# ActiveVisionLab/DFNet

Hardware: AMD Instinct MI355X
Metric: rendered rays/sec (64+128 samples, 640x480) (higher is better)
Workload: dtype f16x3; 1 GPU; BASELINE configs[1]: synthetic random-weight NeRF-H (D=8, W=128), 640x480, 64+128 samples, test-time render_image, 1 frame per step per GPU; parallelism=frames sharded over 1 GPU(s), gather at end, collectives=none (one rank)

## Files before the change

### dfnet_amd/csrc/nerfh_api.hip

```cpp
#include <hip/hip_runtime.h>

#include <cmath>
#include <cstdarg>
#include <cstdio>
#include <cstdlib>
#include <cstring>
#include <map>
#include <string>
#include <type_traits>
#include <vector>

#include "../../include/dfnet_hip.h"
#include "dfn_common.h"
#include "nerfh_fused_train.h"
#include "nerfh_handle.h"
#include "nerfh_kernels.h"
#include "nerfh_layout.h"

using namespace dfn;

namespace dfn {
static thread_local char g_err[512] = "";
int set_error(int code, const char* fmt, ...) {
  va_list ap;
  va_start(ap, fmt);
  vsnprintf(g_err, sizeof g_err, fmt, ap);
  va_end(ap);
  return code;
}
int device_cu_count() {
  static int n = 0;
  if (!n) {
    int dev = 0;
    hipDeviceProp_t p;
    if (hipGetDevice(&dev) == hipSuccess && hipGetDeviceProperties(&p, dev) == hipSuccess) n = p.multiProcessorCount;
    if (n <= 0) n = 256;
  }
  return n;
}
}

extern "C" const char* dfn_last_error(void) { return g_err; }
extern "C" int dfn_abi_version(void) { return 1; }

static std::map<std::string, std::vector<size_t>> expected_shapes(const dfn_nerfh_desc& d) {
  std::map<std::string, std::vector<size_t>> m;
  const size_t W = d.width, na = size_t(d.hist_bin) * d.dim_a, nt = size_t(d.hist_bin) * d.dim_t;
  for (int f = 0; f < 2; ++f) {
    const std::string pre = f ? "fine." : "coarse.";
    for (int i = 0; i < d.depth; ++i) {
      const size_t k = i == 0 ? kChXyz : (i == 4 ? W + kChXyz : W);
      m[pre + "xyz_encoding_" + std::to_string(i + 1) + ".0.weight"] = {W, k};
      m[pre + "xyz_encoding_" + std::to_string(i + 1) + ".0.bias"] = {W};
    }
    m[pre + "xyz_encoding_final.weight"] = {W, W};
    m[pre + "xyz_encoding_final.bias"] = {W};
    m[pre + "dir_encoding.0.weight"] = {W / 2, W + kChDir + (f ? na : 0)};
    m[pre + "dir_encoding.0.bias"] = {W / 2};
    m[pre + "static_sigma.0.weight"] = {1, W};
    m[pre + "static_sigma.0.bias"] = {1};
    m[pre + "static_rgb.0.weight"] = {3, W / 2};
    m[pre + "static_rgb.0.bias"] = {3};
    if (f) {
      const size_t ks[4] = {W + nt, W / 2, W / 2, W / 2};
      for (int j = 0; j < 4; ++j) {
        m[pre + "transient_encoding." + std::to_string(2 * j) + ".weight"] = {W / 2, ks[j]};
        m[pre + "transient_encoding." + std::to_string(2 * j) + ".bias"] = {W / 2};
      }
      m[pre + "transient_sigma.0.weight"] = {1, W / 2};
      m[pre + "transient_sigma.0.bias"] = {1};
      m[pre + "transient_rgb.0.weight"] = {3, W / 2};
      m[pre + "transient_rgb.0.bias"] = {3};
      m[pre + "transient_beta.0.weight"] = {1, W / 2};
      m[pre + "transient_beta.0.bias"] = {1};
    }
  }
  m["embedding_a.weight"] = {size_t(d.n_vocab), size_t(d.dim_a)};
  m["embedding_t.weight"] = {size_t(d.n_vocab), size_t(d.dim_t)};
  return m;
}

extern "C" int dfn_nerfh_create(const dfn_nerfh_desc* desc, dfn_nerfh_t* out) {
  if (!desc || !out) return set_error(DFN_ERR_ARG, "dfn_nerfh_create: null argument");
  if (desc->depth != 8 || desc->multires != kLxyz || desc->multires_views != kLdir)
    return set_error(DFN_ERR_UNSUPPORTED,
                     "dfn_nerfh_create: kernels are specialised for netdepth=8 multires=%d multires_views=%d (got %d/%d/%d)",
                     kLxyz, kLdir, desc->depth, desc->multires, desc->multires_views);
  if (desc->width < 2 || desc->width > 1024 || (desc->width & 1))
    return set_error(DFN_ERR_UNSUPPORTED, "dfn_nerfh_create: netwidth must be even and in [2, 1024] (got %d)", desc->width);
  if (desc->hist_bin <= 0 || desc->dim_a <= 0 || desc->dim_t <= 0 || desc->n_vocab <= 0 ||
      desc->hist_bin * (desc->dim_a + desc->dim_t) > 1024)
    return set_error(DFN_ERR_ARG, "dfn_nerfh_create: bad embedding geometry");
  auto* h = new dfn_nerfh_s();
  h->desc = *desc;
  *out = h;
  return DFN_OK;
}

static void free_packed(dfn_nerfh_s* h) {
  for (auto& a : h->net)
    for (auto& b : a)
      for (auto& n : b) {
        if (n.blob) (void)hipFree(n.blob);
        if (n.tab) (void)hipFree(n.tab);
        n = PackedNet();
      }
  for (auto& n : h->bwd) {
    if (n.blob) (void)hipFree(n.blob);
    if (n.tab) (void)hipFree(n.tab);
    n = PackedNet();
  }
  if (h->extra) (void)hipFree(h->extra);
  h->extra = nullptr;
  if (h->gen_blob) (void)hipFree(h->gen_blob);
  h->gen_blob = nullptr;
  h->gen_params.clear();
  h->fast = false;
}

extern "C" int dfn_nerfh_destroy(dfn_nerfh_t h) {
  if (!h) return DFN_OK;
  free_packed(h);
  dfn::fused::destroy_state(h);
  for (hipEvent_t e : h->side_ev) if (e) (void)hipEventDestroy(e);
  if (h->side_stream) (void)hipStreamDestroy(h->side_stream);
  if (h->range_flag) (void)hipFree(h->range_flag);
  delete h;
  return DFN_OK;
}

extern "C" int dfn_nerfh_set_param(dfn_nerfh_t h, const char* name, const float* host, size_t numel) {
  if (!h || !name || !host) return set_error(DFN_ERR_ARG, "dfn_nerfh_set_param: null argument");
  const auto shapes = expected_shapes(h->desc);
  const auto it = shapes.find(name);
  if (it == shapes.end()) return set_error(DFN_ERR_ARG, "dfn_nerfh_set_param: unknown parameter '%s'", name);
  size_t want = 1;
  for (size_t s : it->second) want *= s;
  if (want != numel)
    return set_error(DFN_ERR_ARG, "dfn_nerfh_set_param: '%s' has %zu elements, expected %zu", name, numel, want);
  h->params[name].assign(host, host + numel);
  h->committed = false;
  return DFN_OK;
}

namespace {

struct Mat {
  const float* w = nullptr;
  const float* b = nullptr;
  int rows = 0, cols = 0;
};

struct Packer {
  const dfn_nerfh_s* h;
  std::string pre;
  int width() const { return h->desc.width; }
  mutable int fwd_units = 0;
  std::vector<float> fold_dir, fold_tr;
  Mat mat(const std::string& key) const {
    Mat m;
    const auto& w = h->params.at(pre + key + ".weight");
    const auto& b = h->params.at(pre + key + ".bias");
    m.w = w.data();
    m.b = b.data();
    m.rows = int(b.size());
    m.cols = int(w.size() / b.size());
    return m;
  }
  void row_source(int layer, int mb, int i, Mat& m, int& row) const {
    row = 32 * mb + i;
    switch (layer) {
      case LY_L1: case LY_L2: case LY_L3: case LY_L4: case LY_L5: case LY_L6: case LY_L7: case LY_L8:
        m = mat("xyz_encoding_" + std::to_string(layer - LY_L1 + 1) + ".0");
        break;
      case LY_FIN:
        if (mb < width() / 32) m = mat("xyz_encoding_final");
        else { m = mat("static_sigma.0"); row = i == 0 ? 0 : -1; }
        break;
      case LY_DIR: m = mat("dir_encoding.0"); break;
      case LY_RGB: m = mat("static_rgb.0"); row = i < 3 ? i : -1; break;
      case LY_TE0: m = mat("transient_encoding.0"); break;
      case LY_TE1: m = mat("transient_encoding.2"); break;
      case LY_TE2: m = mat("transient_encoding.4"); break;
      case LY_TE3: m = mat("transient_encoding.6"); break;
      case LY_THEAD:
        if (i < 3) { m = mat("transient_rgb.0"); row = i; }
        else if (i == 3) { m = mat("transient_sigma.0"); row = 0; }
        else if (i == 8) { m = mat("transient_beta.0"); row = 0; }
        else { m = mat("transient_beta.0"); row = -1; }
        break;
      case LY_SIG: m = mat("static_sigma.0"); row = i == 0 ? 0 : -1; break;
      case LY_DIRF: case LY_TE0F:
        m = Mat();
        m.w = (layer == LY_DIRF ? fold_dir : fold_tr).data();
        m.rows = width() / 2;
        m.cols = width();
        break;
    }
  }
  static int col_source(int layer, int hh, int s) {
    if (layer == LY_L1) return pe_xyz_feature(hh, s);
    if (layer == LY_L5) return s < 32 ? pe_xyz_feature(hh, s) : kChXyz + hidden_feature(hh, s - 32);
    return hidden_feature(hh, s);
  }
  static int col_source_m16(int layer, int g, int s) {
    if (layer == LY_L1) return pe_xyz_feature_m16(g, s);
    if (layer == LY_L5) return s < 16 ? pe_xyz_feature_m16(g, s) : kChXyz + hidden_feature_m16(g, s - 16);
    return hidden_feature_m16(g, s);
  }
  bool head_block(int layer, int mb) const {
    return layer == LY_RGB || layer == LY_THEAD || layer == LY_SIG || (layer == LY_FIN && mb == width() / 32);
  }
  int row_m16(int layer, int mb, int i) const { return head_block(layer, mb) ? head_row_m16(i) : i; }
  static bool unit_has_bias(int layer) { return layer != LY_DIR && layer != LY_TE0 && layer != LY_DIRF && layer != LY_TE0F; }

  float wscale = 1.f;
  template <class P>
  void pack_blocks(int layer, int mb0, int group, uint8_t* base) const {
    using Elem = typename std::conditional<P::kSlotsPerChunk == 8, _Float16, float>::type;
    const LayerShape sh = layer_shape(layer, width());
    const int KC = sh.slots / P::kSlotsPerChunk;
    Elem* frag = reinterpret_cast<Elem*>(base);
    float* bias = reinterpret_cast<float*>(base + size_t(group) * KC * 64 * P::kLaneBytes);
    for (int g = 0; g < group; ++g) {
      const int mb = mb0 + g;
      if constexpr (P::kM16) {
        auto source = [&](int i, Mat& m, int& row) {
          const int ri = row_m16(layer, mb, i);
          if (ri < 0) { m = Mat(); row = -1; return; }
          row_source(layer, mb, ri, m, row);
          if (row >= m.rows) row = -1;
        };
        for (int lane = 0; lane < 64; ++lane)
          for (int kc = 0; kc < KC; ++kc) {
            Mat m;
            int row;
            source(16 * (kc & 1) + (lane & 15), m, row);
            for (int j = 0; j < 8; ++j) {
              const int col = col_source_m16(layer, lane >> 4, 8 * (kc >> 1) + j);
              const float v = (row >= 0 && col >= 0 && col < m.cols) ? m.w[size_t(row) * m.cols + col] : 0.f;
              Elem* fr = frag + (size_t(g) * KC + kc) * 64 * 16;
              const Elem hi = Elem(v * wscale);
              fr[lane * 8 + j] = hi;
              fr[512 + lane * 8 + j] = Elem(v * wscale - float(hi));
            }
          }
        for (int lg = 0; lg < 4; ++lg)
          for (int ms = 0; ms < 2; ++ms)
            for (int r = 0; r < 4; ++r) {
              Mat m;
              int row;
              source(16 * ms + 4 * lg + r, m, row);
              const float b = (row >= 0 && unit_has_bias(layer)) ? m.b[row] : 0.f;
              bias[g * 32 + lg * 8 + ms * 4 + r] = b * wscale * kX3ActScale;
            }
        continue;
      }
      for (int lane = 0; lane < 64; ++lane) {
        const int i = lane & 31, hh = lane >> 5;
        Mat m;
        int row;
        row_source(layer, mb, i, m, row);
        if (row >= m.rows) row = -1;
        for (int kc = 0; kc < KC; ++kc)
          for (int j = 0; j < P::kSlotsPerChunk; ++j) {
            const int col = col_source(layer, hh, kc * P::kSlotsPerChunk + j);
            const float v = (row >= 0 && col >= 0 && col < m.cols) ? m.w[size_t(row) * m.cols + col] : 0.f;
            if constexpr (P::kSplit) {
              Elem* fr = frag + (size_t(g) * KC + kc) * 64 * 16;
              const Elem hi = Elem(v * wscale);
              fr[lane * 8 + j] = hi;
              fr[512 + lane * 8 + j] = Elem(v * wscale - float(hi));
            } else {
              frag[((size_t(g) * KC + kc) * 64 + lane) * P::kSlotsPerChunk + j] = Elem(v);
            }
          }
      }
      for (int hh = 0; hh < 2; ++hh)
        for (int r = 0; r < 16; ++r) {
          Mat m;
          int row;
          row_source(layer, mb, mblock_row(hh, r), m, row);
          if (row >= m.rows) row = -1;
          const float b = (row >= 0 && unit_has_bias(layer)) ? m.b[row] : 0.f;
          bias[(g * 2 + hh) * 16 + r] = P::kSplit ? b * wscale * kX3ActScale : b;
        }
    }
  }
  float bwd_elem(int layer, int mb, int i, int hh, int s) const {
    const int k = 32 * mb + i;
    auto W = [](const Mat& m, int row, int col) {
      return (row >= 0 && row < m.rows && col >= 0 && col < m.cols) ? m.w[size_t(row) * m.cols + col] : 0.f;
    };
    auto pe_col = [&](int blk) { return pe_xyz_feature(mblock_half_of_row(i), 16 * blk + mblock_reg_of_row(i)); };
    const int j = hidden_feature(hh, s);
    switch (layer) {
      case BW_THEAD:
        if (j < 3) return W(mat("transient_rgb.0"), j, k);
        if (j == 3) return W(mat("transient_sigma.0"), 0, k);
        if (j == 8) return W(mat("transient_beta.0"), 0, k);
        return 0.f;
      case BW_TE3: return W(mat("transient_encoding.6"), j, k);
      case BW_TE2: return W(mat("transient_encoding.4"), j, k);
      case BW_TE1: return W(mat("transient_encoding.2"), j, k);
      case BW_RGB: return j < 3 ? W(mat("static_rgb.0"), j, k) : 0.f;
      case BW_FINCAT: {
        const bool dirpart = s >= 32;
        const int jj = hidden_feature(hh, s & 31);
        if (mb < 4) return W(mat(dirpart ? "dir_encoding.0" : "transient_encoding.0"), jj, k);
        if (!dirpart) return 0.f;
        const int c = pe_dir_feature(mblock_half_of_row(i), mblock_reg_of_row(i));
        return c >= 0 ? W(mat("dir_encoding.0"), jj, kWidth + c) : 0.f;
      }
      case BW_FIN:
        if (s < 64) return W(mat("xyz_encoding_final"), j, k);
        return (s == 64 && hh == 0) ? W(mat("static_sigma.0"), 0, k) : 0.f;
      case BW_L5:
        if (mb < 4) return W(mat("xyz_encoding_5.0"), j, kChXyz + k);
        return W(mat("xyz_encoding_5.0"), j, pe_col(mb - 4));
      case BW_L1: return W(mat("xyz_encoding_1.0"), j, pe_col(mb));
      default: {
        const int n = 8 - (layer - BW_L8);
        return W(mat("xyz_encoding_" + std::to_string(n) + ".0"), j, k);
      }
    }
  }
  template <class P>
  void pack_bwd_blocks(int layer, int mb0, int group, uint8_t* base) const {
    using Elem = typename std::conditional<P::kSlotsPerChunk == 8, _Float16, float>::type;
    const LayerShape sh = bwd_layer_shape(layer);
    const int KC = sh.slots / P::kSlotsPerChunk;
    Elem* frag = reinterpret_cast<Elem*>(base);
    for (int g = 0; g < group; ++g)
      for (int lane = 0; lane < 64; ++lane)
        for (int kc = 0; kc < KC; ++kc)
          for (int j = 0; j < P::kSlotsPerChunk; ++j) {
            const float v = bwd_elem(layer, mb0 + g, lane & 31, lane >> 5, kc * P::kSlotsPerChunk + j);
            if constexpr (P::kSplit) {
              Elem* fr = frag + (size_t(g) * KC + kc) * 64 * 16;
              const Elem hi = Elem(v * wscale);
              fr[lane * 8 + j] = hi;
              fr[512 + lane * 8 + j] = Elem(v * wscale - float(hi));
            } else {
              frag[((size_t(g) * KC + kc) * 64 + lane) * P::kSlotsPerChunk + j] = Elem(v);
            }
          }
  }
  template <class PF, class P>
  void pack_bwd(std::vector<uint8_t>& blob, std::vector<uint32_t>& tab) const {
    pack<PF>(true, bwd_fwd_unit_mb<PF>(), false, blob, tab);
    fwd_units = int(tab.size() / 2);
    const int umb = bwd_unit_mb<P>();
    for (int layer = 0; layer < BW_COUNT; ++layer) {
      const LayerShape sh = bwd_layer_shape(layer);
      for (int u0 = 0; u0 < sh.mb; u0 += umb) {
        const int mb0 = (umb <= 2 && layer == BW_L5) ? (u0 < 2 ? 4 + u0 : u0 - 2) : u0;
        const int group = sh.mb - mb0 < umb ? sh.mb - mb0 : umb;
        const uint32_t bytes = unit_bytes<P>(sh.slots, group);
        const uint32_t off = uint32_t(blob.size());
        blob.resize(off + bytes, 0);
        tab.push_back(off);
        tab.push_back(bytes);
        pack_bwd_blocks<P>(layer, mb0, group, blob.data() + off);
      }
    }
  }

  template <class P>
  uint32_t blocks_bytes(int layer, int group) const {
    const LayerShape sh = layer_shape(layer, width());
    return uint32_t(group) * (sh.slots / P::kSlotsPerChunk) * 64 * P::kLaneBytes + uint32_t(group) * 128;
  }

  template <class P>
  void pack(bool fine, int umb, bool merge, std::vector<uint8_t>& blob, std::vector<uint32_t>& tab, int l5_umb = -1, bool fold = false) const {
    const int* seq = fine ? (fold ? kFineFoldSeq : kFineSeq) : kCoarseSeq;
    const int* grp = fine ? kFineGroup : kCoarseGroup;
    const int nl = fine ? kFineLayers : kCoarseLayers;
    if (merge) {
      for (int li = 0; li < nl;) {
        int lj = li;
        uint32_t bytes = 0;
        while (lj < nl && grp[lj] == grp[li]) bytes += blocks_bytes<P>(seq[lj], layer_shape(seq[lj], width()).mb), ++lj;
        if (seq[li] == LY_L5) {
          const LayerShape sh = layer_shape(LY_L5, width());
          const int g = l5_unit_mb(umb);
          for (int mb0 = 0; mb0 < sh.mb; mb0 += g) {
            const uint32_t ub = unit_bytes<P>(sh.slots, g), uo = uint32_t(blob.size());
            blob.resize(uo + ub, 0);
            tab.push_back(uo);
            tab.push_back(ub);
            pack_blocks<P>(LY_L5, mb0, g, blob.data() + uo);
          }
          li = lj;
          continue;
        }
        const uint32_t off = uint32_t(blob.size());
        blob.resize(off + align_piece(bytes), 0);
        tab.push_back(off);
        tab.push_back(align_piece(bytes));
        uint32_t at = off;
        for (int l = li; l < lj; ++l) {
          pack_blocks<P>(seq[l], 0, layer_shape(seq[l], width()).mb, blob.data() + at);
          at += blocks_bytes<P>(seq[l], layer_shape(seq[l], width()).mb);
        }
        li = lj;
      }
      return;
    }
    for (int li = 0; li < nl; ++li) {
      const LayerShape sh = layer_shape(seq[li], width());
      const int lu = (seq[li] == LY_L5 && l5_umb > 0) ? l5_umb : umb;
      for (int mb0 = 0; mb0 < sh.mb; mb0 += lu) {
        const int group = sh.mb - mb0 < lu ? sh.mb - mb0 : lu;
        const uint32_t bytes = unit_bytes<P>(sh.slots, group);
        const uint32_t off = uint32_t(blob.size());
        blob.resize(off + bytes, 0);
        tab.push_back(off);
        tab.push_back(bytes);
        pack_blocks<P>(seq[li], mb0, group, blob.data() + off);
      }
    }
  }
};

void fold_final(const std::vector<float>& a, int rows, int lda, const std::vector<float>& F, const std::vector<float>& bF, int W,
                std::vector<float>& af, std::vector<float>& ab) {
  af.assign(size_t(rows) * W, 0.f);
  ab.assign(rows, 0.f);
  std::vector<double> acc(W);
  for (int r = 0; r < rows; ++r) {
    std::fill(acc.begin(), acc.end(), 0.0);
    double b = 0.0;
    for (int k = 0; k < W; ++k) {
      const double ark = a[size_t(r) * lda + k];
      const float* frow = &F[size_t(k) * W];
      for (int c = 0; c < W; ++c) acc[c] += ark * double(frow[c]);
      b += ark * double(bF[k]);
    }
    for (int c = 0; c < W; ++c) af[size_t(r) * W + c] = float(acc[c]);
    ab[r] = float(b);
  }
}

int upload(const void* src, size_t bytes, void** dst) {
  if (hipMalloc(dst, bytes ? bytes : 16) != hipSuccess) return set_error(DFN_ERR_HIP, "hipMalloc(%zu) failed", bytes);
  if (bytes && hipMemcpy(*dst, src, bytes, hipMemcpyHostToDevice) != hipSuccess)
    return set_error(DFN_ERR_HIP, "hipMemcpy H2D (%zu bytes) failed", bytes);
  return DFN_OK;
}

}

__global__ void range_fetch_kernel(int* flag) { flag[1] = atomicExch(flag, 0); }

extern "C" int dfn_nerfh_set_render_options(dfn_nerfh_t h, int flags) {
  if (!h) return set_error(DFN_ERR_ARG, "dfn_nerfh_set_render_options: null handle");
  if (flags & ~(DFN_RENDER_LINDISP | DFN_RENDER_COARSE_F16)) return set_error(DFN_ERR_UNSUPPORTED, "dfn_nerfh_set_render_options: unknown option bits 0x%x", flags);
  h->render_flags = flags;
  return DFN_OK;
}

extern "C" int dfn_nerfh_range_status(dfn_nerfh_t h, int* flags, void* stream) {
  if (!h) return set_error(DFN_ERR_ARG, "dfn_nerfh_range_status: null handle");
  int v = 0;
  if (h->range_flag) {
    hipStream_t s = static_cast<hipStream_t>(stream);
    hipLaunchKernelGGL(range_fetch_kernel, dim3(1), dim3(1), 0, s, h->range_flag);
    if (hipGetLastError() != hipSuccess || hipMemcpyAsync(&v, h->range_flag + 1, sizeof(int), hipMemcpyDeviceToHost, s) != hipSuccess ||
        hipStreamSynchronize(s) != hipSuccess)
      return set_error(DFN_ERR_HIP, "dfn_nerfh_range_status: reading the flag failed");
  }
  if (flags) { *flags = v; return DFN_OK; }
  if (v)
    return set_error(DFN_ERR_RANGE, "NeRF-H render: activations left the range of the %s arithmetic since the last check (%s); the frames rendered "
                     "since then are not the network's output: render them with DFN_PREC_F32",
                     (v & DFN_RANGE_F16_OVERFLOW) ? "f16" : "split-f16",
                     (v & DFN_RANGE_F16_OVERFLOW) ? "an f16 layer output overflowed to inf: |activation| > 65504"
                                                  : "a split-f16 hi half saturated: |activation| >= 4094 (hidden layers of the render kernels: "
                                                    ">= 4094 x the network's largest |weight|, the accumulators are narrowed before they are scaled)");
  return DFN_OK;
}

extern "C" int dfn_nerfh_range_status_async(dfn_nerfh_t h, int* host_flags, void* stream) {
  if (!h || !host_flags) return set_error(DFN_ERR_ARG, "dfn_nerfh_range_status_async: null handle / destination");
  if (!h->range_flag) { *host_flags = 0; return DFN_OK; }
  hipStream_t s = static_cast<hipStream_t>(stream);
  hipLaunchKernelGGL(range_fetch_kernel, dim3(1), dim3(1), 0, s, h->range_flag);
  if (hipGetLastError() != hipSuccess || hipMemcpyAsync(host_flags, h->range_flag + 1, sizeof(int), hipMemcpyDeviceToHost, s) != hipSuccess)
    return set_error(DFN_ERR_HIP, "dfn_nerfh_range_status_async: enqueueing the read failed");
  return DFN_OK;
}

extern "C" int dfn_nerfh_commit(dfn_nerfh_t h) {
  if (!h) return set_error(DFN_ERR_ARG, "dfn_nerfh_commit: null handle");
  for (const auto& kv : expected_shapes(h->desc))
    if (!h->params.count(kv.first)) return set_error(DFN_ERR_STATE, "dfn_nerfh_commit: parameter '%s' not set", kv.first.c_str());
  free_packed(h);
  dfn::fused::destroy_state(h);
  if (!h->range_flag) {
    if (hipMalloc(reinterpret_cast<void**>(&h->range_flag), 3 * sizeof(int)) != hipSuccess) {
      h->range_flag = nullptr;
      return set_error(DFN_ERR_HIP, "dfn_nerfh_commit: allocating the range-guard flag failed");
    }
    if (hipMemset(h->range_flag, 0, 3 * sizeof(int)) != hipSuccess) return set_error(DFN_ERR_HIP, "dfn_nerfh_commit: clearing the range-guard flag failed");
  }
  {
    std::vector<float> all;
    std::vector<size_t> offs;
    const int np = dfn_nerfh_train_param_count();
    for (int i = 0; i < np; ++i) {
      const auto& v = h->params.at(dfn_nerfh_train_param_name(i));
      offs.push_back(all.size());
      all.insert(all.end(), v.begin(), v.end());
      all.resize((all.size() + 3) & ~size_t(3));
    }
    int rc = upload(all.data(), all.size() * 4, reinterpret_cast<void**>(&h->gen_blob));
    if (rc) return rc;
    for (size_t o : offs) h->gen_params.push_back(h->gen_blob + o);
  }
  const int Wd = h->desc.width;
  std::vector<float> fold_bd, fold_bt;
  if (Wd != kWidth && Wd != kMaxWidth) {
    h->committed = true;
    return DFN_OK;
  }
  if (Wd == kMaxWidth) {
    for (int f = 0; f < 2; ++f)
      for (int prec = 0; prec < 3; ++prec) {
        Packer pk{h, f ? "fine." : "coarse."};
        std::vector<uint8_t> blob;
        std::vector<uint32_t> tab;
        PackedNet& n = h->net[f][prec][0];
        if (prec == DFN_PREC_F16) pk.pack<PrecF16>(f, unit_mb_w256<PrecF16>(), false, blob, tab);
        else if (prec == DFN_PREC_F32) pk.pack<PrecF32>(f, unit_mb_w256<PrecF32>(), false, blob, tab);
        else {
          float wmax = 0.f;
          for (const auto& kv : h->params)
            if (kv.first.compare(0, pk.pre.size(), pk.pre) == 0 && kv.first.find(".weight") != std::string::npos)
              for (float v : kv.second) wmax = std::fmax(wmax, std::fabs(v));
          int sexp = wmax > 0.f ? -int(std::ceil(std::log2(wmax))) : 0;
          sexp = sexp < -8 ? -8 : (sexp > 24 ? 24 : sexp);
          pk.wscale = std::ldexp(1.f, sexp);
          n.in_scale = pk.wscale * kX3ActScale;
          pk.pack<PrecX3>(f, unit_mb_w256<PrecX3>(), false, blob, tab);
        }
        int rc = upload(blob.data(), blob.size(), reinterpret_cast<void**>(&n.blob));
        if (rc) return rc;
        rc = upload(tab.data(), tab.size() * 4, reinterpret_cast<void**>(&n.tab));
        if (rc) return rc;
        n.n_units = int(tab.size() / 2);
      }
  } else {
  for (int f = 0; f < 2; ++f)
    for (int prec = 0; prec < 3; ++prec)
      for (int var = 0; var < kVariants; ++var) {
        const bool fold = var == kFoldVariant;
        if (fold && !(f == 1 && prec == DFN_PREC_F16X3)) continue;
        Packer pk{h, f ? "fine." : "coarse."};
        std::vector<uint8_t> blob;
        std::vector<uint32_t> tab;
        PackedNet& n = h->net[f][prec][var];
        if (prec == DFN_PREC_F16) pk.pack<PrecF16>(f, unit_mb<PrecF16>(var), unit_mb<PrecF16>(var) >= 8, blob, tab);
        else if (prec == DFN_PREC_F32) pk.pack<PrecF32>(f, unit_mb<PrecF32>(var), false, blob, tab);
        else {
          float wmax = 0.f;
          for (const auto& kv : h->params)
            if (kv.first.compare(0, pk.pre.size(), pk.pre) == 0 && kv.first.find(".weight") != std::string::npos)
              for (float v : kv.second) wmax = std::fmax(wmax, std::fabs(v));
          int sexp = wmax > 0.f ? -int(std::ceil(std::log2(wmax))) : 0;
          sexp = sexp < -8 ? -8 : (sexp > 24 ? 24 : sexp);
          pk.wscale = std::ldexp(1.f, sexp);
          n.in_scale = pk.wscale * kX3ActScale;
          if (fold) {
            const int ldd = Wd + kChDir + h->desc.hist_bin * h->desc.dim_a, ldt = Wd + h->desc.hist_bin * h->desc.dim_t;
            const auto& F = h->params.at("fine.xyz_encoding_final.weight");
            const auto& bF = h->params.at("fine.xyz_encoding_final.bias");
            fold_final(h->params.at("fine.dir_encoding.0.weight"), Wd / 2, ldd, F, bF, Wd, pk.fold_dir, fold_bd);
            fold_final(h->params.at("fine.transient_encoding.0.weight"), Wd / 2, ldt, F, bF, Wd, pk.fold_tr, fold_bt);
            pk.pack<PrecX3M16>(f, unit_mb<PrecX3M16>(var), false, blob, tab, l5_unit_mb_p<PrecX3M16>(unit_mb<PrecX3M16>(var)), true);
          } else if (var == 4) pk.pack<PrecX3M16>(f, unit_mb<PrecX3M16>(var), false, blob, tab, l5_unit_mb_p<PrecX3M16>(unit_mb<PrecX3M16>(var)));
          else pk.pack<PrecX3>(f, unit_mb<PrecX3>(var), false, blob, tab, l5_unit_mb_p<PrecX3>(unit_mb<PrecX3>(var)));
        }
        int rc = upload(blob.data(), blob.size(), reinterpret_cast<void**>(&n.blob));
        if (rc) return rc;
        rc = upload(tab.data(), tab.size() * 4, reinterpret_cast<void**>(&n.tab));
        if (rc) return rc;
        n.n_units = int(tab.size() / 2);
      }
  for (int prec = 0; prec < 3; ++prec) {
    Packer pk{h, "fine."};
    std::vector<uint8_t> blob;
    std::vector<uint32_t> tab;
    PackedNet& n = h->bwd[prec];
    if (prec == DFN_PREC_F16) pk.pack_bwd<PrecF16, PrecF16>(blob, tab);
    else if (prec == DFN_PREC_F32) pk.pack_bwd<PrecF32, PrecF32>(blob, tab);
    else {
      n.in_scale = h->net[1][2][0].in_scale * 1024.f;
      pk.wscale = n.in_scale / kX3ActScale;
      pk.pack_bwd<PrecX3, PrecX3>(blob, tab);
    }
    int rc = upload(blob.data(), blob.size(), reinterpret_cast<void**>(&n.blob));
    if (rc) return rc;
    rc = upload(tab.data(), tab.size() * 4, reinterpret_cast<void**>(&n.tab));
    if (rc) return rc;
    n.n_units = int(tab.size() / 2);
    n.n_fwd_units = pk.fwd_units;
  }
  }
  const dfn_nerfh_desc& d = h->desc;
  const int na = d.hist_bin * d.dim_a, nt = d.hist_bin * d.dim_t, kd = kChDir + na, NO = Wd / 2;
  const auto& wd = h->params.at("fine.dir_encoding.0.weight");
  const auto& bd = h->params.at("fine.dir_encoding.0.bias");
  const auto& wt = h->params.at("fine.transient_encoding.0.weight");
  const auto& bt = h->params.at("fine.transient_encoding.0.bias");
  const auto& ea = h->params.at("embedding_a.weight");
  const auto& et = h->params.at("embedding_t.weight");
  std::vector<float> ex;
  const size_t o_wd = 0, o_bd = o_wd + size_t(kd) * NO, o_wt = o_bd + NO, o_bt = o_wt + size_t(nt) * NO,
               o_ea = o_bt + NO, o_et = o_ea + ea.size(), o_bdf = o_et + et.size(), o_btf = o_bdf + NO;
  ex.resize(o_btf + NO);
  const int ld_d = Wd + kd, ld_t = Wd + nt;
  for (int j = 0; j < kd; ++j)
    for (int f = 0; f < NO; ++f) ex[o_wd + size_t(j) * NO + f] = wd[size_t(f) * ld_d + Wd + j];
  for (int j = 0; j < nt; ++j)
    for (int f = 0; f < NO; ++f) ex[o_wt + size_t(j) * NO + f] = wt[size_t(f) * ld_t + Wd + j];
  std::memcpy(&ex[o_bd], bd.data(), NO * 4);
  std::memcpy(&ex[o_bt], bt.data(), NO * 4);
  std::memcpy(&ex[o_ea], ea.data(), ea.size() * 4);
  std::memcpy(&ex[o_et], et.data(), et.size() * 4);
  for (int f = 0; f < NO; ++f) {
    ex[o_bdf + f] = fold_bd.empty() ? bd[f] : bd[f] + fold_bd[f];
    ex[o_btf + f] = fold_bt.empty() ? bt[f] : bt[f] + fold_bt[f];
  }
  int rc = upload(ex.data(), ex.size() * 4, reinterpret_cast<void**>(&h->extra));
  if (rc) return rc;
  h->rb.w_dir = h->extra + o_wd;
  h->rb.b_dir = h->extra + o_bd;
  h->rb.w_tr = h->extra + o_wt;
  h->rb.b_tr = h->extra + o_bt;
  h->rb.emb_a = h->extra + o_ea;
  h->rb.emb_t = h->extra + o_et;
  h->rb.hist_bin = d.hist_bin;
  h->rb.dim_a = d.dim_a;
  h->rb.dim_t = d.dim_t;
  h->rb.n_vocab = d.n_vocab;
  h->rb.nout = NO;
  h->rb_fold = h->rb;
  h->rb_fold.b_dir = h->extra + o_bdf;
  h->rb_fold.b_tr = h->extra + o_btf;
  h->committed = true;
  h->fast = true;
  return DFN_OK;
}

namespace {
struct KernelTimer {
  bool on = false;
  std::vector<std::pair<hipEvent_t, hipEvent_t>> ev[DFN_PROF_SLOTS];
} g_prof;
struct ScopedTimer {
  int which;
  hipStream_t s;
  hipEvent_t a = nullptr, b = nullptr;
  ScopedTimer(int w, hipStream_t st) : which(w), s(st) {
    if (!g_prof.on) return;
    (void)hipEventCreate(&a);
    (void)hipEventCreate(&b);
    (void)hipEventRecord(a, s);
  }
  ~ScopedTimer() {
    if (!a) return;
    (void)hipEventRecord(b, s);
    g_prof.ev[which].emplace_back(a, b);
  }
};
}

extern "C" int dfn_profile_enable(int on) {
  for (auto& v : g_prof.ev) {
    for (auto& p : v) { (void)hipEventDestroy(p.first); (void)hipEventDestroy(p.second); }
    v.clear();
  }
  g_prof.on = on != 0;
  return DFN_OK;
}
extern "C" int dfn_profile_read(int which, double* avg_ms, int* launches) {
  if (which < 0 || which >= DFN_PROF_SLOTS || !avg_ms || !launches) return set_error(DFN_ERR_ARG, "dfn_profile_read: bad argument");
  double tot = 0;
  for (auto& p : g_prof.ev[which]) {
    float ms = 0;
    if (hipEventSynchronize(p.second) != hipSuccess || hipEventElapsedTime(&ms, p.first, p.second) != hipSuccess)
      return set_error(DFN_ERR_HIP, "dfn_profile_read: event query failed");
    tot += ms;
  }
  *launches = int(g_prof.ev[which].size());
  *avg_ms = *launches ? tot / *launches : 0.0;
  return DFN_OK;
}

#define HS(s) reinterpret_cast<hipStream_t>(s)
#define CHECK_HIP(expr, what)                                                                   \
  do {                                                                                          \
    hipError_t e_ = (expr);                                                                     \
    if (e_ != hipSuccess) return set_error(DFN_ERR_HIP, "%s: %s", what, hipGetErrorString(e_)); \
  } while (0)

static int check_net(dfn_nerfh_t h, int prec, const char* fn, bool allow_x3 = false) {
  if (!h) return set_error(DFN_ERR_ARG, "%s: null handle", fn);
  if (!h->committed) return set_error(DFN_ERR_STATE, "%s: dfn_nerfh_commit() has not been called", fn);
  if (!h->fast)
    return set_error(DFN_ERR_UNSUPPORTED, "%s: the register-resident kernels exist for netwidth %d and %d (this handle: %d); "
                     "use the generic-width entry points (dfn_nerfh_generic_*)", fn, kWidth, kMaxWidth, h->desc.width);
  if (prec != DFN_PREC_F16 && prec != DFN_PREC_F32 && !(allow_x3 && prec == DFN_PREC_F16X3))
    return set_error(DFN_ERR_ARG, "%s: unknown / unsupported precision %d", fn, prec);
  return DFN_OK;
}

static int check_grad_width(dfn_nerfh_t h, const char* fn) {
  if (h->desc.width != kWidth)
    return set_error(DFN_ERR_UNSUPPORTED, "%s: the input-gradient kernels are built for netwidth %d only (this handle: %d)", fn, kWidth,
                     h->desc.width);
  return DFN_OK;
}
static int check_grad_prec(int prec, const char* fn) {
  if (prec == DFN_PREC_F16)
    return set_error(DFN_ERR_UNSUPPORTED, "%s: gradients run in DFN_PREC_F16X3 or DFN_PREC_F32 only (plain-f16 ReLU gates are 3e-2 off "
                     "autograd)", fn);
  return DFN_OK;
}

static int mlp_variant_128();
static int mlp_variant_of(dfn_nerfh_t h) { return h->desc.width == kWidth ? mlp_variant_128() : 0; }
static int mlp_variant_128() {
  static int v = -1;
  if (v < 0) {
    const char* e = getenv("DFN_MLP_VARIANT");
    v = (e && e[0] >= '0' && e[0] < '0' + kVariants) ? e[0] - '0' : kFoldVariant;
  }
  return v;
}
static int base_variant(int var) { return var == kFoldVariant ? 4 : var; }
static bool fold_fine(int var, int prec) { return var == kFoldVariant && prec == DFN_PREC_F16X3; }

static int* range_flag_of(dfn_nerfh_t h) { return h->range_flag; }

static unsigned long long* g_timing_buf = nullptr;
extern "C" void dfn_debug_set_timing_buffer(void* p) { g_timing_buf = static_cast<unsigned long long*>(p); }


extern "C" int dfn_raygen(int H, int W, float focal, const float* c2w, float* rays_o, float* rays_d,
                          float* viewdirs, void* stream) {
  if (H < 0 || W < 0 || !c2w || !rays_o || !rays_d || !(focal > 0)) return set_error(DFN_ERR_ARG, "dfn_raygen: bad argument");
  CHECK_HIP(launch_raygen(H, W, focal, c2w, rays_o, rays_d, viewdirs, HS(stream)), "dfn_raygen");
  return DFN_OK;
}

extern "C" int dfn_posenc(const float* x, size_t n, int L, int mode, float* out, void* stream) {
  if (!x || !out || L < 0 || L > 16 || (mode != 0 && mode != 1)) return set_error(DFN_ERR_ARG, "dfn_posenc: bad argument");
  CHECK_HIP(launch_posenc(x, n, L, mode, out, HS(stream)), "dfn_posenc");
  return DFN_OK;
}

extern "C" int dfn_mlp_coarse(dfn_nerfh_t h, int prec, const float* rays_o, const float* rays_d, size_t n_rays,
                              int Nc, float near, float far, float* sigma, void* stream) {
  if (int rc = check_net(h, prec, "dfn_mlp_coarse", true)) return rc;
  if (!n_rays) return DFN_OK;
  if (!rays_o || !rays_d || !sigma || Nc < 1) return set_error(DFN_ERR_ARG, "dfn_mlp_coarse: bad argument");
  const int var = base_variant(mlp_variant_of(h));
  const PackedNet& n = h->net[0][prec][var];
  MlpArgs a{n.blob, n.tab, n.n_units, rays_o, rays_d, nullptr, nullptr, sigma, nullptr, (long long)n_rays, Nc, near, far, nullptr, n.in_scale,
            h->render_flags & DFN_RENDER_LINDISP};
  a.status = range_flag_of(h);
  ScopedTimer t(0, HS(stream));
  CHECK_HIP(launch_mlp(false, prec, var, a, device_cu_count(), HS(stream), h->desc.width), "dfn_mlp_coarse");
  return DFN_OK;
}

extern "C" int dfn_coarse_weights(const float* sigma, const float* z, size_t n, int N, float* weights, void* stream) {
  if (!sigma || !z || !weights || N < 1 || N > 2048) return set_error(DFN_ERR_ARG, "dfn_coarse_weights: bad argument");
  CHECK_HIP(launch_coarse_weights(sigma, z, n, N, weights, HS(stream)), "dfn_coarse_weights");
  return DFN_OK;
}

extern "C" int dfn_sample_pdf(const float* bins, const float* weights, size_t n, int nb, int Ni, const float* u,
                              float* out, void* stream) {
  if (!bins || !weights || !out || nb < 2 || Ni < 1 || 3 * nb + 2 * Ni > 8192)
    return set_error(DFN_ERR_ARG, "dfn_sample_pdf: bad argument");
  CHECK_HIP(launch_sample_pdf(bins, weights, n, nb, Ni, u, out, HS(stream)), "dfn_sample_pdf");
  return DFN_OK;
}

extern "C" int dfn_sample_fine_opt(const float* sigma, size_t n_rays, int Nc, int Ni, float near, float far, int render_flags,
                                   float* z_fine, float* weights_coarse, float* z_samples, void* stream) {
  if (!sigma || !z_fine || Nc < 3 || Ni < 1 || 6 * Nc + 2 * Ni > 8192)
    return set_error(DFN_ERR_ARG, "dfn_sample_fine: bad argument (need N_samples >= 3, N_importance >= 1)");
  if ((render_flags & DFN_RENDER_LINDISP) && !(near > 0.f))
    return set_error(DFN_ERR_ARG, "dfn_sample_fine: lindisp needs near > 0");
  CHECK_HIP(launch_sample_fine(sigma, n_rays, Nc, Ni, near, far, z_fine, weights_coarse, z_samples, HS(stream),
                               render_flags & DFN_RENDER_LINDISP),
            "dfn_sample_fine");
  return DFN_OK;
}
extern "C" int dfn_sample_fine(const float* sigma, size_t n_rays, int Nc, int Ni, float near, float far,
                               float* z_fine, float* weights_coarse, float* z_samples, void* stream) {
  return dfn_sample_fine_opt(sigma, n_rays, Nc, Ni, near, far, 0, z_fine, weights_coarse, z_samples, stream);
}

extern "C" int dfn_ndc_rays(int H, int W, float focal, float near, const float* rays_o, const float* rays_d, size_t n, float* out_o,
                            float* out_d, void* stream) {
  if (!n) return DFN_OK;
  if (!rays_o || !rays_d || !out_o || !out_d || H < 1 || W < 1 || !(focal > 0.f)) return set_error(DFN_ERR_ARG, "dfn_ndc_rays: bad argument");
  CHECK_HIP(launch_ndc_rays(H, W, focal, near, rays_o, rays_d, n, out_o, out_d, HS(stream)), "dfn_ndc_rays");
  return DFN_OK;
}

extern "C" int dfn_upsample_bicubic(const float* in, int H, int W, int C, int outH, int outW, float* out, void* stream) {
  if (!in || !out || H < 1 || W < 1 || C < 1 || outH < 1 || outW < 1) return set_error(DFN_ERR_ARG, "dfn_upsample_bicubic: bad argument");
  CHECK_HIP(launch_bicubic(in, H, W, C, outH, outW, out, HS(stream)), "dfn_upsample_bicubic");
  return DFN_OK;
}

extern "C" int dfn_upsample_bicubic_frames(const float* in, int B, int H, int W, int C, int outH, int outW, int out_nchw, float* out,
                                           void* stream) {
  if (!in || !out || B < 1 || H < 1 || W < 1 || C < 1 || outH < 1 || outW < 1) return set_error(DFN_ERR_ARG, "dfn_upsample_bicubic_frames: bad argument");
  CHECK_HIP(launch_bicubic(in, H, W, C, outH, outW, out, HS(stream), B, out_nchw != 0), "dfn_upsample_bicubic_frames");
  return DFN_OK;
}
extern "C" int dfn_upsample_bicubic_frames_backward(const float* grad_out, int B, int H, int W, int C, int outH, int outW, int out_nchw,
                                                    float* grad_in, void* stream) {
  if (!grad_out || !grad_in || B < 1 || H < 1 || W < 1 || C < 1 || outH < 1 || outW < 1)
    return set_error(DFN_ERR_ARG, "dfn_upsample_bicubic_frames_backward: bad argument");
  CHECK_HIP(launch_bicubic_backward(grad_out, H, W, C, outH, outW, grad_in, HS(stream), B, out_nchw != 0), "dfn_upsample_bicubic_frames_backward");
  return DFN_OK;
}

extern "C" int dfn_upsample_bicubic_backward(const float* grad_out, int H, int W, int C, int outH, int outW, float* grad_in,
                                             void* stream) {
  if (!grad_out || !grad_in || H < 1 || W < 1 || C < 1 || outH < 1 || outW < 1)
    return set_error(DFN_ERR_ARG, "dfn_upsample_bicubic_backward: bad argument");
  CHECK_HIP(launch_bicubic_backward(grad_out, H, W, C, outH, outW, grad_in, HS(stream)), "dfn_upsample_bicubic_backward");
  return DFN_OK;
}

extern "C" size_t dfn_fine_bias_bytes(size_t n_rays) { return (n_rays ? n_rays : 1) * ray_bias_floats(kMaxWidth) * sizeof(float); }

extern "C" int dfn_mlp_fine(dfn_nerfh_t h, int prec, const float* rays_o, const float* rays_d, const float* viewdirs,
                            const float* hist, size_t hist_rows, size_t n_rays, const float* z_fine, int Nf,
                            float* raw, void* bias_ws, void* stream) {
  if (int rc = check_net(h, prec, "dfn_mlp_fine", true)) return rc;
  if (!n_rays) return DFN_OK;
  if (!rays_o || !rays_d || !viewdirs || !hist || !z_fine || !raw || !bias_ws || Nf < 1 ||
      (hist_rows != 1 && hist_rows != n_rays))
    return set_error(DFN_ERR_ARG, "dfn_mlp_fine: bad argument (hist_rows must be 1 or n_rays)");
  float* table = static_cast<float*>(bias_ws);
  const bool fold = fold_fine(mlp_variant_of(h), prec);
  const int var = fold ? kFoldVariant : base_variant(mlp_variant_of(h));
  CHECK_HIP(launch_ray_bias(fold ? h->rb_fold : h->rb, viewdirs, hist, hist_rows, n_rays, table, HS(stream)), "dfn_mlp_fine(ray_bias)");
  const PackedNet& n = h->net[1][prec][var];
  MlpArgs a{n.blob, n.tab, n.n_units, rays_o, rays_d, z_fine, table, raw, nullptr, (long long)n_rays, Nf, 0.f, 0.f, g_timing_buf, n.in_scale};
  a.status = range_flag_of(h);
  ScopedTimer t(1, HS(stream));
  if (fold) CHECK_HIP(launch_mlp_fold(false, a, device_cu_count(), HS(stream)), "dfn_mlp_fine");
  else CHECK_HIP(launch_mlp(true, prec, var, a, device_cu_count(), HS(stream), h->desc.width), "dfn_mlp_fine");
  return DFN_OK;
}

extern "C" int dfn_composite_fine(const float* raw, const float* z, size_t n_rays, int Nf, float beta_min, int flags,
                                  float* rgb, float* disp, float* acc, float* depth, float* weights, float* beta,
                                  void* stream) {
  if (!raw || !z || !rgb || !disp || !acc || Nf < 1 || Nf > 512)
    return set_error(DFN_ERR_ARG, "dfn_composite_fine: bad argument (1 <= Nf <= 512)");
  CHECK_HIP(launch_composite_fine(raw, z, n_rays, Nf, beta_min, flags, rgb, disp, acc, depth, weights, beta, HS(stream)),
            "dfn_composite_fine");
  return DFN_OK;
}

static MapPtrs map_ptrs(const dfn_render_maps* m) {
  return m ? MapPtrs{m->depth, m->depth_static, m->beta, m->rgb_static, m->rgb_transient} : MapPtrs{};
}

extern "C" int dfn_composite_fine_maps(const float* raw, const float* z, size_t n_rays, int Nf, float beta_min,
                                       const dfn_render_maps* maps, void* stream) {
  if (!raw || !z || Nf < 1 || Nf > 512) return set_error(DFN_ERR_ARG, "dfn_composite_fine_maps: bad argument (1 <= Nf <= 512)");
  CHECK_HIP(launch_composite_fine_maps(raw, z, n_rays, Nf, beta_min, map_ptrs(maps), HS(stream)), "dfn_composite_fine_maps");
  return DFN_OK;
}

namespace {
constexpr size_t kMaxChunkRays = 65536;
inline size_t al(size_t b) { return (b + 255) & ~size_t(255); }
inline size_t chunk_rays(size_t n_rays) {
  const size_t passes = (n_rays + kMaxChunkRays - 1) / kMaxChunkRays;
  const size_t c = passes ? (n_rays + passes - 1) / passes : 1;
  return (c + 63) & ~size_t(63);
}
struct Workspace {
  float *o, *d, *v, *sigma, *z, *raw, *bias, *partial;
  size_t total;
};
Workspace carve(char* base, size_t n_rays, int Nc, int Ni, bool own_rays, int rec_floats = 12) {
  const size_t chunk = chunk_rays(n_rays);
  const size_t Nf = size_t(Nc) + Ni;
  Workspace w{};
  size_t off = 0;
  auto take = [&](size_t bytes) { char* p = base ? base + off : nullptr; off += al(bytes); return reinterpret_cast<float*>(p); };
  w.o = take(own_rays ? n_rays * 12 : 0);
  w.d = take(own_rays ? n_rays * 12 : 0);
  w.v = take(n_rays * 12);
  w.sigma = take(chunk * Nc * 4);
  w.z = take(chunk * Nf * 4);
  w.raw = take(chunk * Nf * 9 * 4);
  w.bias = take(chunk * ray_bias_floats(kMaxWidth) * 4);
  w.partial = take(chunk * ((Nf + 31) / 32) * rec_floats * 4);
  w.total = off;
  return w;
}

int render_core(dfn_nerfh_t h, int prec, const float* o, const float* d, const float* v, const float* hist,
                size_t hist_rows, size_t n_rays, int Nc, int Ni, float near, float far, float* rgb, float* disp,
                float* acc, float* raw_out, const Workspace& w, hipStream_t s, const MapPtrs& maps = MapPtrs{}) {
  const int Nf = Nc + Ni;
  const bool want_maps = maps.any();
  const bool fold = fold_fine(mlp_variant_of(h), prec);
  const int var = base_variant(mlp_variant_of(h));
  const int seg = prec == DFN_PREC_F16 ? 64 : 32;
  const bool fused = !raw_out && Nf % seg == 0 && !(prec == DFN_PREC_F16 && var == 2) && h->desc.width == kWidth;
  const int cprec = (h->render_flags & DFN_RENDER_COARSE_F16) ? DFN_PREC_F16 : prec;
  const PackedNet& nc = h->net[0][cprec][var];
  const PackedNet& nf = h->net[1][prec][fold ? kFoldVariant : var];
  const int cus = device_cu_count();
  const size_t chunk = chunk_rays(n_rays);
  for (size_t r0 = 0; r0 < n_rays; r0 += chunk) {
    const size_t n = n_rays - r0 < chunk ? n_rays - r0 : chunk;
    const float* co = o + r0 * 3;
    const float* cd = d + r0 * 3;
    const float* cv = v + r0 * 3;
    const float* ch = hist_rows == 1 ? hist : hist + r0 * h->desc.hist_bin;
    float* raw = raw_out ? raw_out + r0 * size_t(Nf) * 9 : w.raw;
    {
      MlpArgs a{nc.blob, nc.tab, nc.n_units, co, cd, nullptr, nullptr, w.sigma, nullptr, (long long)n, Nc, near, far, nullptr, nc.in_scale,
                 h->render_flags & DFN_RENDER_LINDISP};
      a.status = range_flag_of(h);
      ScopedTimer t(0, s);
      CHECK_HIP(launch_mlp(false, cprec, var, a, cus, s, h->desc.width), "render: coarse MLP");
    }
    {
      ScopedTimer t(DFN_PROF_SAMPLE_FINE, s);
      CHECK_HIP(launch_sample_fine(w.sigma, n, Nc, Ni, near, far, w.z, nullptr, nullptr, s, h->render_flags & DFN_RENDER_LINDISP),
                "render: sample_fine");
    }
    {
      ScopedTimer t(DFN_PROF_RAY_BIAS, s);
      CHECK_HIP(launch_ray_bias(fold ? h->rb_fold : h->rb, cv, ch, hist_rows, n, w.bias, s), "render: ray_bias");
    }
    {
      MlpArgs a{nf.blob, nf.tab, nf.n_units, co, cd, w.z, w.bias, raw, fused ? w.partial : nullptr, (long long)n, Nf, 0.f, 0.f, g_timing_buf, nf.in_scale};
      a.status = range_flag_of(h);
      ScopedTimer t(1, s);
      if (fold) CHECK_HIP(launch_mlp_fold(fused && want_maps, a, cus, s), "render: fine MLP (folded)");
      else if (fused && want_maps) CHECK_HIP(launch_mlp_maps(true, prec, var, a, cus, s, h->desc.width), "render: fine MLP (maps)");
      else CHECK_HIP(launch_mlp(true, prec, var, a, cus, s, h->desc.width), "render: fine MLP");
    }
    if (fused && want_maps) {
      ScopedTimer t(DFN_PROF_COMBINE, s);
      CHECK_HIP(launch_composite_combine_maps(w.partial, n, Nf / seg, 0.1f, DFN_COMP_TEST_TIME | DFN_COMP_STATIC_ONLY, rgb + r0 * 3,
                                              disp + r0, acc + r0, maps.at(r0), s),
                "render: composite combine (maps)");
    } else if (fused) {
      ScopedTimer t(DFN_PROF_COMBINE, s);
      CHECK_HIP(launch_composite_combine(w.partial, n, Nf / seg, 0.1f, DFN_COMP_TEST_TIME | DFN_COMP_STATIC_ONLY, rgb + r0 * 3,
                                         disp + r0, acc + r0, s),
                "render: composite combine");
    } else {
      ScopedTimer t(DFN_PROF_COMPOSITE, s);
      CHECK_HIP(launch_composite_fine(raw, w.z, n, Nf, 0.1f, DFN_COMP_TEST_TIME | DFN_COMP_STATIC_ONLY, rgb + r0 * 3,
                                      disp + r0, acc + r0, nullptr, nullptr, nullptr, s),
                "render: composite");
      if (want_maps) CHECK_HIP(launch_composite_fine_maps(raw, w.z, n, Nf, 0.1f, maps.at(r0), s), "render: composite (maps)");
    }
  }
  return DFN_OK;
}

int check_render_args(int Nc, int Ni, const char* fn) {
  if (Nc < 3 || Ni < 1 || Nc + Ni > 512 || 6 * Nc + 2 * Ni > 8192)
    return set_error(DFN_ERR_UNSUPPORTED, "%s: need 3 <= N_samples, 1 <= N_importance, N_samples+N_importance <= 512", fn);
  return DFN_OK;
}
}

extern "C" size_t dfn_render_workspace_bytes(size_t n_rays, int Nc, int Ni) {
  return carve(nullptr, n_rays ? n_rays : 1, Nc, Ni, true).total;
}

static int render_rays_entry(const char* fn, dfn_nerfh_t h, int prec, const float* rays_o, const float* rays_d, const float* viewdirs,
                             const float* hist, size_t hist_rows, size_t n_rays, int Nc, int Ni, float near, float far,
                             float* rgb, float* disp, float* acc, float* raw, void* workspace, size_t workspace_bytes,
                             const MapPtrs& maps, void* stream) {
  if (int rc = check_net(h, prec, fn, true)) return rc;
  if (int rc = check_render_args(Nc, Ni, fn)) return rc;
  if (!n_rays) return DFN_OK;
  if (!rays_o || !rays_d || !hist || !rgb || !disp || !acc || !workspace || (hist_rows != 1 && hist_rows != n_rays))
    return set_error(DFN_ERR_ARG, "%s: bad argument (hist_rows must be 1 or n_rays)", fn);
  const Workspace w = carve(static_cast<char*>(workspace), n_rays, Nc, Ni, true, maps.any() ? kMapsRecFloats : 12);
  if (w.total > workspace_bytes)
    return set_error(DFN_ERR_ARG, "%s: workspace too small (%zu < %zu)", fn, workspace_bytes, w.total);
  const float* v = viewdirs;
  if (!v) {
    if (hipError_t e = launch_viewdirs(rays_d, n_rays, w.v, HS(stream)); e != hipSuccess)
      return set_error(DFN_ERR_HIP, "%s: viewdirs: %s", fn, hipGetErrorString(e));
    v = w.v;
  }
  return render_core(h, prec, rays_o, rays_d, v, hist, hist_rows, n_rays, Nc, Ni, near, far, rgb, disp, acc, raw, w,
                     HS(stream), maps);
}

static int render_image_entry(const char* fn, dfn_nerfh_t h, int prec, const float* c2w, int H, int W, float focal, float near,
                              float far, int Nc, int Ni, const float* hist, float* rgb, float* disp, float* acc,
                              void* workspace, size_t workspace_bytes, const MapPtrs& maps, void* stream) {
  if (int rc = check_net(h, prec, fn, true)) return rc;
  if (int rc = check_render_args(Nc, Ni, fn)) return rc;
  if (!c2w || !hist || !rgb || !disp || !acc || !workspace || H < 1 || W < 1 || !(focal > 0))
    return set_error(DFN_ERR_ARG, "%s: bad argument", fn);
  const size_t n_rays = size_t(H) * W;
  const Workspace w = carve(static_cast<char*>(workspace), n_rays, Nc, Ni, true, maps.any() ? kMapsRecFloats : 12);
  if (w.total > workspace_bytes)
    return set_error(DFN_ERR_ARG, "%s: workspace too small (%zu < %zu)", fn, workspace_bytes, w.total);
  if (hipError_t e = launch_raygen(H, W, focal, c2w, w.o, w.d, w.v, HS(stream)); e != hipSuccess)
    return set_error(DFN_ERR_HIP, "%s: raygen: %s", fn, hipGetErrorString(e));
  return render_core(h, prec, w.o, w.d, w.v, hist, 1, n_rays, Nc, Ni, near, far, rgb, disp, acc, nullptr, w, HS(stream), maps);
}

extern "C" int dfn_render_rays(dfn_nerfh_t h, int prec, const float* rays_o, const float* rays_d, const float* viewdirs,
                               const float* hist, size_t hist_rows, size_t n_rays, int Nc, int Ni, float near, float far,
                               float* rgb, float* disp, float* acc, float* raw, void* workspace, size_t workspace_bytes,
                               void* stream) {
  return render_rays_entry("dfn_render_rays", h, prec, rays_o, rays_d, viewdirs, hist, hist_rows, n_rays, Nc, Ni, near, far, rgb, disp,
                           acc, raw, workspace, workspace_bytes, MapPtrs{}, stream);
}

extern "C" int dfn_render_image(dfn_nerfh_t h, int prec, const float* c2w, int H, int W, float focal, float near,
                                float far, int Nc, int Ni, const float* hist, float* rgb, float* disp, float* acc,
                                void* workspace, size_t workspace_bytes, void* stream) {
  return render_image_entry("dfn_render_image", h, prec, c2w, H, W, focal, near, far, Nc, Ni, hist, rgb, disp, acc, workspace,
                            workspace_bytes, MapPtrs{}, stream);
}

extern "C" size_t dfn_render_maps_workspace_bytes(size_t n_rays, int Nc, int Ni) {
  return carve(nullptr, n_rays ? n_rays : 1, Nc, Ni, true, kMapsRecFloats).total;
}

extern "C" int dfn_render_rays_maps(dfn_nerfh_t h, int prec, const float* rays_o, const float* rays_d, const float* viewdirs,
                                    const float* hist, size_t hist_rows, size_t n_rays, int Nc, int Ni, float near, float far,
                                    float* rgb, float* disp, float* acc, float* raw, void* workspace, size_t workspace_bytes,
                                    const dfn_render_maps* maps, void* stream) {
  return render_rays_entry("dfn_render_rays_maps", h, prec, rays_o, rays_d, viewdirs, hist, hist_rows, n_rays, Nc, Ni, near, far, rgb,
                           disp, acc, raw, workspace, workspace_bytes, map_ptrs(maps), stream);
}

extern "C" int dfn_render_image_maps(dfn_nerfh_t h, int prec, const float* c2w, int H, int W, float focal, float near,
                                     float far, int Nc, int Ni, const float* hist, float* rgb, float* disp, float* acc,
                                     void* workspace, size_t workspace_bytes, const dfn_render_maps* maps, void* stream) {
  return render_image_entry("dfn_render_image_maps", h, prec, c2w, H, W, focal, near, far, Nc, Ni, hist, rgb, disp, acc, workspace,
                            workspace_bytes, map_ptrs(maps), stream);
}

extern "C" int dfn_composite_fine_backward(const float* raw, const float* z, const float* grad_rgb, size_t n_rays, int Nf,
                                           float* grad_raw, void* stream) {
  if (!raw || !z || !grad_rgb || !grad_raw || Nf < 1 || Nf > 512)
    return set_error(DFN_ERR_ARG, "dfn_composite_fine_backward: bad argument (1 <= Nf <= 512)");
  CHECK_HIP(launch_composite_fine_backward(raw, z, grad_rgb, n_rays, Nf, grad_raw, HS(stream)), "dfn_composite_fine_backward");
  return DFN_OK;
}

extern "C" int dfn_composite_fine_backward_maps(const float* raw, const float* z, size_t n_rays, int Nf, float beta_min,
                                                const dfn_map_grads* grads, const float* grad_raw_ext, float* grad_raw, void* stream) {
  if (!raw || !z || !grad_raw || Nf < 1 || Nf > 512)
    return set_error(DFN_ERR_ARG, "dfn_composite_fine_backward_maps: bad argument (1 <= Nf <= 512)");
  const MapGrads g = grads ? MapGrads{grads->rgb, grads->acc, grads->depth, grads->depth_static, grads->disp, grads->beta,
                                      grads->rgb_static, grads->rgb_transient}
                           : MapGrads{};
  if (!g.any() && !grad_raw_ext)
    return set_error(DFN_ERR_ARG, "dfn_composite_fine_backward_maps: bad argument (no upstream gradient and no grad_raw_ext)");
  CHECK_HIP(launch_composite_fine_backward_all(raw, z, n_rays, Nf, beta_min, g, grad_raw, HS(stream), grad_raw_ext),
            "dfn_composite_fine_backward_maps");
  return DFN_OK;
}

extern "C" int dfn_mlp_fine_backward(dfn_nerfh_t h, int prec, const float* rays_o, const float* rays_d, const float* viewdirs,
                                     const float* hist, size_t hist_rows, size_t n_rays, const float* z_fine, int Nf,
                                     const float* grad_raw, float* grad_pts, void* bias_ws, void* stream) {
  if (int rc = check_net(h, prec, "dfn_mlp_fine_backward", true)) return rc;
  if (int rc = check_grad_prec(prec, "dfn_mlp_fine_backward")) return rc;
  if (int rc = check_grad_width(h, "dfn_mlp_fine_backward")) return rc;
  if (!n_rays) return DFN_OK;
  if (!rays_o || !rays_d || !viewdirs || !hist || !z_fine || !grad_raw || !grad_pts || !bias_ws || Nf < 1 ||
      (hist_rows != 1 && hist_rows != n_rays))
    return set_error(DFN_ERR_ARG, "dfn_mlp_fine_backward: bad argument (hist_rows must be 1 or n_rays)");
  float* table = static_cast<float*>(bias_ws);
  CHECK_HIP(launch_ray_bias(h->rb, viewdirs, hist, hist_rows, n_rays, table, HS(stream)), "dfn_mlp_fine_backward(ray_bias)");
  const PackedNet& n = h->bwd[prec];
  BwdArgs a{n.blob, n.tab, n.n_units, rays_o, rays_d, viewdirs, z_fine, table, grad_raw, grad_pts, (long long)n_rays, Nf, n.in_scale};
  CHECK_HIP(launch_mlp_fine_backward(prec, a, device_cu_count(), HS(stream)), "dfn_mlp_fine_backward");
  return DFN_OK;
}

extern "C" size_t dfn_mlp_fine_mask_bytes(size_t n_points) {
  return (n_points + kBwdTilePoints - 1) / kBwdTilePoints * (kBwdTilePoints / 32) * kBwdMaskWords * 64 * sizeof(uint32_t);
}

extern "C" int dfn_mlp_fine_saving(dfn_nerfh_t h, int prec, const float* rays_o, const float* rays_d, const float* viewdirs,
                                   const float* hist, size_t hist_rows, size_t n_rays, const float* z_fine, int Nf, float* raw,
                                   void* masks, void* bias_ws, void* stream) {
  if (int rc = check_net(h, prec, "dfn_mlp_fine_saving", true)) return rc;
  if (int rc = check_grad_width(h, "dfn_mlp_fine_saving")) return rc;
  if (prec != DFN_PREC_F16X3) return set_error(DFN_ERR_UNSUPPORTED, "dfn_mlp_fine_saving: split-f16 (DFN_PREC_F16X3) only");
  if (!n_rays) return DFN_OK;
  if (!rays_o || !rays_d || !viewdirs || !hist || !z_fine || !raw || !masks || !bias_ws || Nf < 1 ||
      (hist_rows != 1 && hist_rows != n_rays))
    return set_error(DFN_ERR_ARG, "dfn_mlp_fine_saving: bad argument (hist_rows must be 1 or n_rays)");
  float* table = static_cast<float*>(bias_ws);
  CHECK_HIP(launch_ray_bias(h->rb, viewdirs, hist, hist_rows, n_rays, table, HS(stream)), "dfn_mlp_fine_saving(ray_bias)");
  const PackedNet& n = h->net[1][prec][0];
  MlpArgs a{n.blob, n.tab, n.n_units, rays_o, rays_d, z_fine, table, raw, nullptr, (long long)n_rays, Nf, 0.f, 0.f, nullptr, n.in_scale};
  a.status = range_flag_of(h);
  a.masks = static_cast<uint32_t*>(masks);
  CHECK_HIP(launch_mlp(true, prec, 0, a, device_cu_count(), HS(stream), h->desc.width), "dfn_mlp_fine_saving");
  return DFN_OK;
}

extern "C" int dfn_mlp_fine_backward_saved(dfn_nerfh_t h, int prec, const float* rays_o, const float* rays_d, const float* viewdirs,
                                           size_t n_rays, const float* z_fine, int Nf, const float* raw, const void* masks,
                                           const float* grad_raw, float* grad_pts, void* stream) {
  if (int rc = check_net(h, prec, "dfn_mlp_fine_backward_saved", true)) return rc;
  if (int rc = check_grad_width(h, "dfn_mlp_fine_backward_saved")) return rc;
  if (prec != DFN_PREC_F16X3) return set_error(DFN_ERR_UNSUPPORTED, "dfn_mlp_fine_backward_saved: split-f16 (DFN_PREC_F16X3) only");
  if (!n_rays) return DFN_OK;
  if (!rays_o || !rays_d || !viewdirs || !z_fine || !raw || !masks || !grad_raw || !grad_pts || Nf < 1)
    return set_error(DFN_ERR_ARG, "dfn_mlp_fine_backward_saved: bad argument");
  const PackedNet& n = h->bwd[prec];
  BwdArgs a{n.blob, n.tab + 2 * n.n_fwd_units, n.n_units - n.n_fwd_units, rays_o, rays_d, viewdirs, z_fine, nullptr, grad_raw, grad_pts,
            (long long)n_rays, Nf, n.in_scale, nullptr, raw, static_cast<uint32_t*>(const_cast<void*>(masks))};
  CHECK_HIP(launch_mlp_fine_backward(prec, a, device_cu_count(), HS(stream), 2), "dfn_mlp_fine_backward_saved");
  return DFN_OK;
}

extern "C" int dfn_ray_grad_reduce(const float* grad_pts, const float* z_fine, const float* rays_d, size_t n_rays, int Nf,
                                   int derive_viewdirs, float* grad_rays_o, float* grad_rays_d, float* grad_viewdirs,
                                   void* stream) {
  if (!grad_pts || !z_fine || !rays_d || !grad_rays_o || !grad_rays_d || Nf < 1)
    return set_error(DFN_ERR_ARG, "dfn_ray_grad_reduce: bad argument");
  CHECK_HIP(launch_ray_grad_reduce(grad_pts, z_fine, rays_d, n_rays, Nf, derive_viewdirs, grad_rays_o, grad_rays_d, grad_viewdirs,
                                   HS(stream)),
            "dfn_ray_grad_reduce");
  return DFN_OK;
}

extern "C" int dfn_raygen_frames(int B, int H, int W, float focal, const float* c2w, float* rays_o, float* rays_d, float* viewdirs,
                                 void* stream) {
  if (B < 1 || H < 0 || W < 0 || !c2w || !rays_o || !rays_d || !(focal > 0)) return set_error(DFN_ERR_ARG, "dfn_raygen_frames: bad argument");
  CHECK_HIP(launch_raygen(H, W, focal, c2w, rays_o, rays_d, viewdirs, HS(stream), B), "dfn_raygen_frames");
  return DFN_OK;
}
extern "C" int dfn_raygen_frames_backward(int B, int H, int W, float focal, const float* grad_rays_o, const float* grad_rays_d,
                                          float* grad_c2w, void* stream) {
  if (B < 1 || H < 1 || W < 1 || !grad_rays_o || !grad_rays_d || !grad_c2w || !(focal > 0))
    return set_error(DFN_ERR_ARG, "dfn_raygen_frames_backward: bad argument");
  CHECK_HIP(launch_raygen_backward(H, W, focal, grad_rays_o, grad_rays_d, grad_c2w, HS(stream), B), "dfn_raygen_frames_backward");
  return DFN_OK;
}

extern "C" int dfn_raygen_backward(int H, int W, float focal, const float* grad_rays_o, const float* grad_rays_d, float* grad_c2w,
                                   void* stream) {
  if (H < 1 || W < 1 || !(focal > 0) || !grad_rays_o || !grad_rays_d || !grad_c2w)
    return set_error(DFN_ERR_ARG, "dfn_raygen_backward: bad argument");
  CHECK_HIP(launch_raygen_backward(H, W, focal, grad_rays_o, grad_rays_d, grad_c2w, HS(stream)), "dfn_raygen_backward");
  return DFN_OK;
}

namespace {
struct BwdWorkspace {
  Workspace f;
  float *graw, *gpts, *go, *gd;
  size_t total;
};
BwdWorkspace carve_bwd(char* base, size_t n_rays, int Nc, int Ni) {
  BwdWorkspace b{};
  b.f = carve(base, n_rays, Nc, Ni, true);
  const size_t chunk = chunk_rays(n_rays), Nf = size_t(Nc) + Ni;
  size_t off = b.f.total;
  auto take = [&](size_t bytes) { char* p = base ? base + off : nullptr; off += al(bytes); return reinterpret_cast<float*>(p); };
  b.graw = take(chunk * Nf * 9 * 4);
  b.gpts = take(chunk * Nf * 6 * 4);
  b.go = take(n_rays * 12);
  b.gd = take(n_rays * 12);
  b.total = off;
  return b;
}

int render_backward_core(dfn_nerfh_t h, int prec, const float* o, const float* d, const float* v, bool derive_v,
                         const float* hist, size_t hist_rows, size_t n_rays, int Nc, int Ni, float near, float far,
                         const float* grad_rgb, float* go, float* gd, float* gv, const BwdWorkspace& w, hipStream_t s) {
  const int Nf = Nc + Ni, var = base_variant(mlp_variant_of(h)), cus = device_cu_count();
  const PackedNet& nc = h->net[0][prec][var];
  const PackedNet& nf = h->net[1][prec][var];
  const PackedNet& nb = h->bwd[prec];
  const size_t chunk = chunk_rays(n_rays);
  for (size_t r0 = 0; r0 < n_rays; r0 += chunk) {
    const size_t n = n_rays - r0 < chunk ? n_rays - r0 : chunk;
    const float* co = o + r0 * 3;
    const float* cd = d + r0 * 3;
    const float* cv = v + r0 * 3;
    const float* ch = hist_rows == 1 ? hist : hist + r0 * h->desc.hist_bin;
    MlpArgs ac{nc.blob, nc.tab, nc.n_units, co, cd, nullptr, nullptr, w.f.sigma, nullptr, (long long)n, Nc, near, far, nullptr, nc.in_scale,
                 h->render_flags & DFN_RENDER_LINDISP};
    ac.status = range_flag_of(h);
    CHECK_HIP(launch_mlp(false, prec, var, ac, cus, s, h->desc.width), "render backward: coarse MLP");
    CHECK_HIP(launch_sample_fine(w.f.sigma, n, Nc, Ni, near, far, w.f.z, nullptr, nullptr, s, h->render_flags & DFN_RENDER_LINDISP),
              "render backward: sample_fine");
    CHECK_HIP(launch_ray_bias(h->rb, cv, ch, hist_rows, n, w.f.bias, s), "render backward: ray_bias");
    MlpArgs af{nf.blob, nf.tab, nf.n_units, co, cd, w.f.z, w.f.bias, w.f.raw, nullptr, (long long)n, Nf, 0.f, 0.f, nullptr, nf.in_scale};
    af.status = range_flag_of(h);
    CHECK_HIP(launch_mlp(true, prec, var, af, cus, s, h->desc.width), "render backward: fine MLP");
    CHECK_HIP(launch_composite_fine_backward(w.f.raw, w.f.z, grad_rgb + r0 * 3, n, Nf, w.graw, s), "render backward: composite");
    BwdArgs ab{nb.blob, nb.tab, nb.n_units, co, cd, cv, w.f.z, w.f.bias, w.graw, w.gpts, (long long)n, Nf, nb.in_scale};
    CHECK_HIP(launch_mlp_fine_backward(prec, ab, cus, s), "render backward: fine MLP gradient");
    CHECK_HIP(launch_ray_grad_reduce(w.gpts, w.f.z, cd, n, Nf, derive_v ? 1 : 0, go + r0 * 3, gd + r0 * 3,
                                     gv ? gv + r0 * 3 : nullptr, s),
              "render backward: ray reduction");
  }
  return DFN_OK;
}
}

extern "C" size_t dfn_render_backward_workspace_bytes(size_t n_rays, int Nc, int Ni) {
  return carve_bwd(nullptr, n_rays ? n_rays : 1, Nc, Ni).total;
}

extern "C" int dfn_render_rays_backward(dfn_nerfh_t h, int prec, const float* rays_o, const float* rays_d, const float* viewdirs,
                                        const float* hist, size_t hist_rows, size_t n_rays, int Nc, int Ni, float near,
                                        float far, const float* grad_rgb, float* grad_rays_o, float* grad_rays_d,
                                        float* grad_viewdirs, void* workspace, size_t workspace_bytes, void* stream) {
  if (int rc = check_net(h, prec, "dfn_render_rays_backward", true)) return rc;
  if (int rc = check_grad_prec(prec, "dfn_render_rays_backward")) return rc;
  if (int rc = check_grad_width(h, "dfn_render_rays_backward")) return rc;
  if (int rc = check_render_args(Nc, Ni, "dfn_render_rays_backward")) return rc;
  if (!n_rays) return DFN_OK;
  if (!rays_o || !rays_d || !hist || !grad_rgb || !grad_rays_o || !grad_rays_d || !workspace ||
      (hist_rows != 1 && hist_rows != n_rays))
    return set_error(DFN_ERR_ARG, "dfn_render_rays_backward: bad argument (hist_rows must be 1 or n_rays)");
  if (!n_rays) return DFN_OK;
  const BwdWorkspace w = carve_bwd(static_cast<char*>(workspace), n_rays, Nc, Ni);
  if (w.total > workspace_bytes)
    return set_error(DFN_ERR_ARG, "dfn_render_rays_backward: workspace too small (%zu < %zu)", workspace_bytes, w.total);
  const float* v = viewdirs;
  if (!v) {
    CHECK_HIP(launch_viewdirs(rays_d, n_rays, w.f.v, HS(stream)), "dfn_render_rays_backward: viewdirs");
    v = w.f.v;
  }
  return render_backward_core(h, prec, rays_o, rays_d, v, viewdirs == nullptr, hist, hist_rows, n_rays, Nc, Ni, near, far,
                              grad_rgb, grad_rays_o, grad_rays_d, viewdirs ? grad_viewdirs : nullptr, w, HS(stream));
}

extern "C" int dfn_render_image_backward(dfn_nerfh_t h, int prec, const float* c2w, int H, int W, float focal, float near,
                                         float far, int Nc, int Ni, const float* hist, const float* grad_rgb,
                                         float* grad_c2w, void* workspace, size_t workspace_bytes, void* stream) {
  if (int rc = check_net(h, prec, "dfn_render_image_backward", true)) return rc;
  if (int rc = check_grad_prec(prec, "dfn_render_image_backward")) return rc;
  if (int rc = check_grad_width(h, "dfn_render_image_backward")) return rc;
  if (int rc = check_render_args(Nc, Ni, "dfn_render_image_backward")) return rc;
  if (!c2w || !hist || !grad_rgb || !grad_c2w || !workspace || H < 1 || W < 1 || !(focal > 0))
    return set_error(DFN_ERR_ARG, "dfn_render_image_backward: bad argument");
  const size_t n_rays = size_t(H) * W;
  const BwdWorkspace w = carve_bwd(static_cast<char*>(workspace), n_rays, Nc, Ni);
  if (w.total > workspace_bytes)
    return set_error(DFN_ERR_ARG, "dfn_render_image_backward: workspace too small (%zu < %zu)", workspace_bytes, w.total);
  CHECK_HIP(launch_raygen(H, W, focal, c2w, w.f.o, w.f.d, w.f.v, HS(stream)), "dfn_render_image_backward: raygen");
  if (int rc = render_backward_core(h, prec, w.f.o, w.f.d, w.f.v, true, hist, 1, n_rays, Nc, Ni, near, far, grad_rgb, w.go,
                                    w.gd, nullptr, w, HS(stream)))
    return rc;
  CHECK_HIP(launch_raygen_backward(H, W, focal, w.go, w.gd, grad_c2w, HS(stream)), "dfn_render_image_backward: raygen");
  return DFN_OK;
}
```

### dfnet_amd/csrc/nerfh_handle.h

```cpp
#pragma once
#include <map>
#include <string>
#include <vector>

#include "../../include/dfnet_hip.h"
#include "nerfh_kernels.h"
#include "nerfh_layout.h"

struct PackedNet {
  char* blob = nullptr;
  uint32_t* tab = nullptr;
  int n_units = 0;
  int n_fwd_units = 0;
  float in_scale = 1.f;
};

struct dfn_nerfh_s {
  dfn_nerfh_desc desc;
  std::map<std::string, std::vector<float>> params;
  bool committed = false;
  PackedNet net[2][3][dfn::kVariants];
  PackedNet bwd[3];
  float* extra = nullptr;
  dfn::RayBiasWeights rb{};
  dfn::RayBiasWeights rb_fold{};
  bool fast = false;
  float* gen_blob = nullptr;
  std::vector<const float*> gen_params;
  int render_flags = 0;
  int* range_flag = nullptr;
  void* fused = nullptr;
  bool train_forward_exact = false;
  bool train_split_fine = false;
  bool train_forward_split = false;
  bool train_exact = false;
  hipStream_t side_stream = nullptr;
  hipEvent_t side_ev[2] = {nullptr, nullptr};
};
```

### dfnet_amd/csrc/nerfh_kernels.h

```cpp
#pragma once
#include <hip/hip_runtime.h>
#include <stddef.h>
#include <stdint.h>

namespace dfn {

struct MlpArgs {
  const char* blob;
  const uint32_t* tab;
  int n_units;
  const float* rays_o;
  const float* rays_d;
  const float* z;
  const float* ray_bias;
  float* out;
  float* partial;
  long long n_rays;
  int n_samples;
  float near, far;
  unsigned long long* timing;
  float in_scale;
  int lindisp;
  int dma_waves;
  int* status;
  uint32_t* masks;
};

constexpr int kMapsRecFloats = 16;
hipError_t launch_mlp(bool fine, int prec, int variant, const MlpArgs& a, int n_cu, hipStream_t stream, int width = 128);
hipError_t launch_mlp_maps(bool fine, int prec, int variant, const MlpArgs& a, int n_cu, hipStream_t stream, int width = 128);
hipError_t launch_mlp_fold(bool maps, const MlpArgs& a, int n_cu, hipStream_t stream);

hipError_t launch_raygen(int H, int W, float focal, const float* c2w, float* rays_o, float* rays_d,
                         float* viewdirs, hipStream_t stream, int frames = 1);
hipError_t launch_viewdirs(const float* rays_d, size_t n, float* viewdirs, hipStream_t stream);
hipError_t launch_ndc_rays(int H, int W, float focal, float near, const float* rays_o, const float* rays_d, size_t n, float* out_o,
                           float* out_d, hipStream_t stream);
hipError_t launch_posenc(const float* x, size_t n, int L, int mode, float* out, hipStream_t stream);

struct RayBiasWeights {
  const float* w_dir;
  const float* b_dir;
  const float* w_tr;
  const float* b_tr;
  const float* emb_a;
  const float* emb_t;
  int hist_bin, dim_a, dim_t, n_vocab;
  int nout;
};
hipError_t launch_ray_bias(const RayBiasWeights& w, const float* viewdirs, const float* hist,
                           size_t hist_rows, size_t n_rays, float* table, hipStream_t stream);

hipError_t launch_coarse_weights(const float* sigma, const float* z, size_t n, int N, float* weights,
                                 hipStream_t stream);
hipError_t launch_sample_pdf(const float* bins, const float* weights, size_t n, int nb, int Ni,
                             const float* u, float* out, hipStream_t stream);
hipError_t launch_sample_fine(const float* sigma, size_t n_rays, int Nc, int Ni, float near, float far,
                              float* z_fine, float* weights_coarse, float* z_samples, hipStream_t stream, int lindisp = 0);
hipError_t launch_composite_fine(const float* raw, const float* z, size_t n_rays, int Nf, float beta_min,
                                 int flags, float* rgb, float* disp, float* acc, float* depth,
                                 float* weights, float* beta, hipStream_t stream);

hipError_t launch_composite_combine(const float* partial, size_t n_rays, int segs, float beta_min, int flags, float* rgb,
                                    float* disp, float* acc, hipStream_t stream);

struct MapPtrs {
  float *depth, *depth_static, *beta, *rgb_static, *rgb_transient;
  bool any() const { return depth || depth_static || beta || rgb_static || rgb_transient; }
  MapPtrs at(size_t ray) const {
    return MapPtrs{depth ? depth + ray : nullptr, depth_static ? depth_static + ray : nullptr, beta ? beta + ray : nullptr,
                   rgb_static ? rgb_static + ray * 3 : nullptr, rgb_transient ? rgb_transient + ray * 3 : nullptr};
  }
};
hipError_t launch_composite_fine_maps(const float* raw, const float* z, size_t n_rays, int Nf, float beta_min, const MapPtrs& maps,
                                      hipStream_t stream);
hipError_t launch_composite_combine_maps(const float* partial, size_t n_rays, int segs, float beta_min, int flags, float* rgb,
                                         float* disp, float* acc, const MapPtrs& maps, hipStream_t stream);

struct BwdArgs {
  const char* blob;
  const uint32_t* tab;
  int n_units;
  const float* rays_o;
  const float* rays_d;
  const float* viewdirs;
  const float* z;
  const float* ray_bias;
  const float* graw;
  float* gpts;
  long long n_rays;
  int n_samples;
  float in_scale;
  float* raw_out;
  const float* raw_in;
  uint32_t* masks;
};
constexpr int kBwdMaskWords = 21;
constexpr int kBwdTilePoints = 256;
hipError_t launch_mlp_fine_backward(int prec, const BwdArgs& a, int n_cu, hipStream_t stream, int mode = 0);
hipError_t launch_composite_fine_backward(const float* raw, const float* z, const float* grad_rgb, size_t n_rays, int Nf,
                                          float* graw, hipStream_t stream, const float* grad_raw_ext = nullptr);
struct MapGrads {
  const float *rgb, *acc, *depth, *depth_static, *disp, *beta, *rgb_static, *rgb_transient;
  bool any() const { return rgb || acc || depth || depth_static || disp || beta || rgb_static || rgb_transient; }
};
hipError_t launch_composite_fine_backward_all(const float* raw, const float* z, size_t n_rays, int Nf, float beta_min, const MapGrads& g,
                                              float* graw, hipStream_t stream, const float* grad_raw_ext = nullptr);
hipError_t launch_ray_grad_reduce(const float* gpts, const float* z, const float* rays_d, size_t n_rays, int Nf,
                                  int derive_viewdirs, float* grad_o, float* grad_d, float* grad_viewdirs,
                                  hipStream_t stream, int accumulate = 0);
hipError_t launch_raygen_backward(int H, int W, float focal, const float* grad_o, const float* grad_d, float* grad_c2w,
                                  hipStream_t stream, int frames = 1);
hipError_t launch_bicubic_backward(const float* gout, int H, int W, int C, int UH, int UW, float* gin, hipStream_t stream, int frames = 1,
                                   bool nchw = false);
hipError_t launch_bicubic(const float* in, int H, int W, int C, int UH, int UW, float* out, hipStream_t stream, int frames = 1,
                          bool nchw = false);

}
```

### dfnet_amd/csrc/nerfh_layout.h

```cpp
#pragma once
#include <stdint.h>

#if defined(__HIPCC__) || defined(__HIP__)
#define DFN_HD __host__ __device__
#else
#define DFN_HD
#endif

namespace dfn {

constexpr int kWidth = 128;
constexpr int kLxyz = 10;
constexpr int kLdir = 4;
constexpr int kChXyz = 63, kChDir = 27;

enum LayerId {
  LY_L1 = 0, LY_L2, LY_L3, LY_L4, LY_L5, LY_L6, LY_L7, LY_L8,
  LY_FIN,
  LY_DIR,
  LY_RGB,
  LY_TE0,
  LY_TE1, LY_TE2, LY_TE3,
  LY_THEAD,
  LY_SIG,
  LY_DIRF,
  LY_TE0F,
  LY_COUNT
};

struct LayerShape { int slots; int mb; };

DFN_HD constexpr LayerShape layer_shape(int id, int W = kWidth) {
  return id == LY_L1 ? LayerShape{32, W / 32}
       : id == LY_L5 ? LayerShape{32 + W / 2, W / 32}
       : id <= LY_L8 ? LayerShape{W / 2, W / 32}
       : id == LY_FIN ? LayerShape{W / 2, W / 32 + 1}
       : id == LY_DIR ? LayerShape{W / 2, W / 64}
       : id == LY_RGB ? LayerShape{W / 4, 1}
       : id == LY_TE0 ? LayerShape{W / 2, W / 64}
       : id <= LY_TE3 ? LayerShape{W / 4, W / 64}
       : id == LY_THEAD ? LayerShape{W / 4, 1}
       : id == LY_DIRF || id == LY_TE0F ? LayerShape{W / 2, W / 64}
       : LayerShape{W / 2, 1};
}

constexpr int kCoarseSeq[] = {LY_L1, LY_L2, LY_L3, LY_L4, LY_L5, LY_L6, LY_L7, LY_L8, LY_SIG};
constexpr int kFineSeq[] = {LY_L1, LY_L2, LY_L3, LY_L4, LY_L5, LY_L6, LY_L7, LY_L8, LY_FIN,
                            LY_DIR, LY_RGB, LY_TE0, LY_TE1, LY_TE2, LY_TE3, LY_THEAD};
constexpr int kFineFoldSeq[] = {LY_L1, LY_L2, LY_L3, LY_L4, LY_L5, LY_L6, LY_L7, LY_L8, LY_SIG,
                                LY_DIRF, LY_RGB, LY_TE0F, LY_TE1, LY_TE2, LY_TE3, LY_THEAD};
static_assert(sizeof(kFineFoldSeq) == sizeof(kFineSeq), "the folded sequence has the layer count of the plain one");
constexpr int kCoarseGroup[] = {0, 1, 2, 3, 4, 5, 6, 7, 7};
constexpr int kFineGroup[] = {0, 1, 2, 3, 4, 5, 6, 7, 8, 9, 9, 10, 10, 10, 10, 10};
constexpr int kCoarseLayers = sizeof(kCoarseSeq) / sizeof(int);
constexpr int kFineLayers = sizeof(kFineSeq) / sizeof(int);

DFN_HD constexpr int hidden_feature(int h, int s) {
  return 32 * (s >> 4) + 4 * h + (s & 3) + 8 * ((s & 15) >> 2);
}
DFN_HD constexpr int mblock_row(int h, int r) { return (r & 3) + 8 * (r >> 2) + 4 * h; }

DFN_HD constexpr int pe_xyz_feature(int h, int s) {
  return s < 30 ? 3 + 6 * (5 * h + s / 6) + (s % 6) : (s == 30 ? (h ? 2 : 0) : (h ? -1 : 1));
}

DFN_HD constexpr int hidden_feature_m16(int g, int s) { return 32 * (s >> 3) + 16 * ((s & 7) >> 2) + 4 * g + (s & 3); }
DFN_HD constexpr int pe_xyz_feature_m16(int g, int s) {
  return s < 12 ? 3 + 6 * (2 * g + s / 6) + (s % 6)
       : (g == 3 ? (s < 15 ? s - 12 : -1)
                 : 3 + 6 * (8 + (2 * g + ((s - 12) >> 1)) / 3) + 3 * ((s - 12) & 1) + (2 * g + ((s - 12) >> 1)) % 3);
}
DFN_HD constexpr int head_row_m16(int i) {
  return ((i >> 2) & 3) < 2 ? (i & 3) + 8 * (i >> 4) : -1;
}

struct PrecF16 { static constexpr int kSlotsPerChunk = 8, kLaneBytes = 16; static constexpr bool kSplit = false, kM16 = false; };
struct PrecF32 { static constexpr int kSlotsPerChunk = 1, kLaneBytes = 4; static constexpr bool kSplit = false, kM16 = false; };
struct PrecX3 { static constexpr int kSlotsPerChunk = 8, kLaneBytes = 32; static constexpr bool kSplit = true, kM16 = false; };
constexpr float kX3ActScale = 16.f;
struct PrecX3M16 { static constexpr int kSlotsPerChunk = 8, kLaneBytes = 32; static constexpr bool kSplit = true, kM16 = true; };

constexpr int kVariants = 6;
constexpr int kFoldVariant = 5;
template <class P> DFN_HD constexpr int unit_mb(int variant) {
  return P::kSlotsPerChunk == 1 ? 1 : (P::kSplit ? 2 : (variant == 1 ? 2 : 8));
}
DFN_HD constexpr int variant_waves(int variant) { return variant == 0 ? 8 : 4; }
template <class P> DFN_HD constexpr int unit_mb_w256() { return (P::kSlotsPerChunk == 1 || P::kSplit) ? 1 : 2; }

constexpr uint32_t kPiece = 1024;

DFN_HD constexpr uint32_t align_piece(uint32_t b) { return (b + kPiece - 1) / kPiece * kPiece; }

template <class P>
DFN_HD constexpr uint32_t unit_bytes(int slots, int nmb) {
  return align_piece(uint32_t(nmb) * (slots / P::kSlotsPerChunk) * 64 * P::kLaneBytes + uint32_t(nmb) * 2 * 16 * 4);
}
DFN_HD constexpr int l5_unit_mb(int umb) { return umb >= 8 ? 2 : umb; }
template <class P> DFN_HD constexpr int l5_unit_mb_p(int umb) { return (P::kSplit && umb == 2) ? 1 : l5_unit_mb(umb); }
template <class P>
DFN_HD constexpr uint32_t max_unit_bytes(int umb, int W = kWidth) {
  const int m5 = l5_unit_mb_p<P>(umb), mbw = W / 32;
  const uint32_t a = unit_bytes<P>(32 + W / 2, m5 < mbw ? m5 : mbw), b = unit_bytes<P>(W / 2, umb < mbw + 1 ? umb : mbw + 1);
  const uint32_t g = umb >= 8 ? align_piece(44u * 64 * P::kLaneBytes + 9u * 128) : 0;
  return a > b ? (a > g ? a : g) : (b > g ? b : g);
}

enum BwdLayerId {
  BW_THEAD = 0,
  BW_TE3, BW_TE2, BW_TE1,
  BW_RGB,
  BW_FINCAT,
  BW_FIN,
  BW_L8, BW_L7, BW_L6,
  BW_L5,
  BW_L4, BW_L3, BW_L2,
  BW_L1,
  BW_COUNT
};
DFN_HD constexpr LayerShape bwd_layer_shape(int id) {
  return id == BW_THEAD || id == BW_RGB ? LayerShape{16, 2}
       : id <= BW_TE1 ? LayerShape{32, 2}
       : id == BW_FINCAT ? LayerShape{64, 5}
       : id == BW_FIN ? LayerShape{80, 4}
       : id == BW_L5 ? LayerShape{64, 6}
       : id == BW_L1 ? LayerShape{64, 2}
       : LayerShape{64, 4};
}
DFN_HD constexpr int mblock_half_of_row(int i) { return (i >> 2) & 1; }
DFN_HD constexpr int mblock_reg_of_row(int i) { return (i & 3) + 4 * (i >> 3); }
DFN_HD constexpr int pe_dir_feature(int h, int r) {
  return r < 12 ? 3 + 6 * (2 * h + r / 6) + (r % 6) : (h == 0 && r < 15 ? r - 12 : -1);
}
template <class P> DFN_HD constexpr int bwd_fwd_unit_mb() { return (P::kSlotsPerChunk == 8 && !P::kSplit) ? 8 : (P::kSplit ? 2 : 1); }
template <class P> DFN_HD constexpr int bwd_unit_mb() { return (P::kSlotsPerChunk == 8 && !P::kSplit) ? 8 : (P::kSplit ? 2 : 1); }
template <class P>
DFN_HD constexpr uint32_t bwd_max_unit_bytes() {
  constexpr bool whole = P::kSlotsPerChunk == 8 && !P::kSplit;
  constexpr int uf = bwd_fwd_unit_mb<P>(), ub = bwd_unit_mb<P>();
  const uint32_t a = unit_bytes<P>(96, whole ? 4 : uf);
  const uint32_t f5 = unit_bytes<P>(64, whole ? 5 : uf);
  const uint32_t b = unit_bytes<P>(64, whole ? 6 : ub), c = unit_bytes<P>(80, whole ? 4 : ub);
  const uint32_t m1 = a > f5 ? a : f5, m2 = b > c ? b : c;
  return m1 > m2 ? m1 : m2;
}

constexpr int kRayBiasFloats = 2 * 2 * 2 * 16;
DFN_HD constexpr int ray_bias_floats(int W) { return W; }
constexpr int kMaxWidth = 256;

}
```

### dfnet_amd/csrc/nerfh_mlp.hip

```cpp
#include <hip/hip_runtime.h>
#include <stdint.h>
#include <stdlib.h>

#include "nerfh_device.h"
#include "nerfh_kernels.h"
#include "nerfh_layout.h"
#include "mfma_frag.h"

#include "nerfh_mlp_core.h"
#include "nerfh_mask.h"

namespace dfn {

#ifdef DFN_MLP_MAPS_TU
constexpr bool kMapsTU = true;
#define DFN_LAUNCH_MLP launch_mlp_maps
#else
constexpr bool kMapsTU = false;
#define DFN_LAUNCH_MLP launch_mlp
#endif
#ifdef DFN_MLP_FOLD_TU
#define DFN_FINE_KERNEL nerfh_fine_fold_kernel
#else
#define DFN_FINE_KERNEL nerfh_fine_kernel
#endif

template <class P, bool FAST> DFN_DEV float head_softplus(float v) { return FAST ? softplus_fast(v) : (P::kSplit ? softplus_hw(v) : softplus(v)); }
template <class P, bool FAST> DFN_DEV float head_sigmoid(float v) { return FAST ? sigmoid_fast(v) : (P::kSplit ? sigmoid_hw(v) : sigmoid(v)); }
template <class P, bool FAST> DFN_DEV float head_exp(float v) { return FAST ? __expf(v) : (P::kSplit ? exp_hw(v) : expf(v)); }

template <class P, int W> constexpr uint32_t ring_slots() { return 3; }
template <class P, int UMB, int WAVES, int NB, int W = kWidth> constexpr uint32_t lds_bytes() {
  return ring_slots<P, W>() * max_unit_bytes<P>(UMB, W) + WAVES * ((NB * 32 + 63) / 64) * 8 * 256;
}

template <class P, int WAVES, int NB, int W> constexpr int mlp_min_blocks() {
  if (W > kWidth && (P::kSplit || P::kSlotsPerChunk == 1 || NB >= 2)) return 1;
  return WAVES * NB >= 12 ? (WAVES == 8 ? 2 : 1) : 2;
}

template <class P, bool FAST, int WAVES, int UMB, int NB, bool PIPE, int W = kWidth>
__global__ __launch_bounds__(WAVES * 64, (mlp_min_blocks<P, WAVES, NB, W>())) void nerfh_coarse_kernel(MlpArgs a) {
  extern __shared__ __attribute__((aligned(16))) char smem[];
  constexpr int PPT = WAVES * NB * 32;
  using F = typename FragOf<P>::type;
  Stager st;
  st.blob = a.blob; st.tab = a.tab; st.n_units = a.n_units; st.u = 0;
  st.waves = WAVES;
  st.dma_waves = a.dma_waves > 0 && a.dma_waves < WAVES ? a.dma_waves : WAVES;
  st.in_scale = a.in_scale;
  st.out_scale = 1.f / a.in_scale;
  st.lane_mul = 1.f;
  st.rmax = 0;
  st.t_sync = st.t_wait = 0;
  st.trace = nullptr;
  st.n_trace = 0;
  st.lane = threadIdx.x & 63;
  st.wave = __builtin_amdgcn_readfirstlane(threadIdx.x >> 6);
#ifdef DFN_TIMING
  const unsigned long long t_begin = __builtin_amdgcn_s_memtime();
  unsigned long long t_pro = 0;
  if (a.timing && blockIdx.x == 7) st.trace = a.timing + 8192 * 4 + st.wave * 192;
#endif
  const int p = st.lane & 31, h = st.lane >> 5;
  const long long n_pts = (long long)a.n_rays * a.n_samples;
  const long long n_tiles = (n_pts + PPT - 1) / PPT;
  long long tile = blockIdx.x;
  if (tile >= n_tiles) return;
  stage_prime(st, smem, max_unit_bytes<P>(UMB, W), ring_slots<P, W>());
  for (; tile < n_tiles; tile += gridDim.x) {
    st.more = tile + gridDim.x < n_tiles;
    constexpr int LP = lane_pts<P>(NB);
    float x[LP][3];
    uint32_t pt[NB];
    const uint32_t npts = uint32_t(n_pts);
#pragma unroll
    for (int nb = 0; nb < NB; ++nb) pt[nb] = uint32_t(tile) * uint32_t(PPT) + st.wave * (NB * 32) + nb * 32 + p;
#pragma unroll
    for (int n = 0; n < LP; ++n) {
      const uint32_t pn = P::kM16 ? uint32_t(tile) * uint32_t(PPT) + st.wave * 32 + 16 * n + (st.lane & 15) : pt[n];
      const uint32_t q = pn < npts ? pn : npts - 1;
      const uint32_t ray = q / uint32_t(a.n_samples);
      const int i = int(q - ray * uint32_t(a.n_samples));
      const float z = coarse_z_at(i, a.n_samples, a.near, a.far, a.lindisp != 0);
#pragma unroll
      for (int c = 0; c < 3; ++c)
        x[n][c] = add_rn(a.rays_o[ray * 3 + c], mul_rn(a.rays_d[ray * 3 + c], z));
    }
    constexpr bool CY = PIPE && P::kSlotsPerChunk == 8, MERGE = UMB >= 8;
    F hid[NB][chunks_of<P>(W / 2)];
    f32x16 carry[NB];
    trunk<P, UMB, PIPE, FAST, NB, W>(st, smem, x, hid, carry);
    f32x16 head[NB];
    F dummy[NB][chunks_of<P>(16)];
    const float* const norb[LP] = {};
    layer<P, UMB, PIPE, NB, chunks_of<P>(W / 2), 0, false, true, false, !MERGE, (CY ? 6 : -1), true, false>(st, smem, hid, dummy, head, norb, carry);
#pragma unroll
    for (int nb = 0; nb < NB; ++nb)
      if (h == 0 && pt[nb] < npts) a.out[pt[nb]] = head_softplus<P, FAST>(head[nb][0]);
  }
  range_report<P>(st.rmax, a.status);
}

template <class P, bool FAST, int WAVES, int UMB, int NB, bool PIPE, int W = kWidth, bool MASKS = false, bool MAPS = false>
__global__ __launch_bounds__(WAVES * 64, (mlp_min_blocks<P, WAVES, NB, W>())) void DFN_FINE_KERNEL(MlpArgs a) {
  static_assert(!MASKS || (P::kSplit && !P::kM16 && NB == 1 && WAVES == 8 && W == kWidth), "the sign masks follow the gradient kernel's tile geometry");
  static_assert(!MAPS || (!MASKS && W == kWidth && NB <= 2), "the maps flavour exists where the fused compositing does");
  extern __shared__ __attribute__((aligned(16))) char smem[];
  constexpr int PPT = WAVES * NB * 32;
  constexpr int HC = chunks_of<P>(W / 2), QC = chunks_of<P>(W / 4);
  constexpr int MBW = W / 32, MBQ = W / 64;
  constexpr uint32_t USTRIDE = max_unit_bytes<P>(UMB, W);
  constexpr int PF_ROUNDS = (NB * 32 + 63) / 64;
  constexpr int LP = lane_pts<P>(NB);
  using F = typename FragOf<P>::type;
  Stager st;
  st.blob = a.blob; st.tab = a.tab; st.n_units = a.n_units; st.u = 0;
  st.waves = WAVES;
  st.dma_waves = a.dma_waves > 0 && a.dma_waves < WAVES ? a.dma_waves : WAVES;
  st.in_scale = a.in_scale;
  st.out_scale = 1.f / a.in_scale;
  st.lane_mul = 1.f;
  st.rmax = 0;
  st.t_sync = st.t_wait = 0;
  st.trace = nullptr;
  st.n_trace = 0;
  st.lane = threadIdx.x & 63;
  st.wave = __builtin_amdgcn_readfirstlane(threadIdx.x >> 6);
#ifdef DFN_TIMING
  const unsigned long long t_begin = __builtin_amdgcn_s_memtime();
  unsigned long long t_pro = 0;
  if (a.timing && blockIdx.x == 7) st.trace = a.timing + 8192 * 4 + st.wave * 192;
#endif
  const int p = st.lane & 31, h = st.lane >> 5;
  const long long n_pts = (long long)a.n_rays * a.n_samples;
  const long long n_tiles = (n_pts + PPT - 1) / PPT;
  long long tile = blockIdx.x;
  if (tile >= n_tiles) return;
  stage_prime(st, smem, USTRIDE, ring_slots<P, W>());
  float zin[LP], znext[LP], oin[LP][3], din[LP][3];
  uint32_t pt[LP], ray_of[LP];
  const uint32_t npts = uint32_t(n_pts);
  auto tile_coords = [&](long long t) {
    uint32_t lp = st.lane;
    asm volatile("" : "+v"(lp));
#pragma unroll
    for (int nb = 0; nb < LP; ++nb) {
      pt[nb] = uint32_t(t) * uint32_t(PPT) + st.wave * (NB * 32) + (P::kM16 ? 16 * nb + (lp & 15) : nb * 32 + (lp & 31));
      const uint32_t q = pt[nb] < npts ? pt[nb] : npts - 1;
      ray_of[nb] = q / uint32_t(a.n_samples);
    }
  };
  tile_coords(tile);
#pragma unroll
  for (int nb = 0; nb < LP; ++nb) {
    const uint32_t q = pt[nb] < npts ? pt[nb] : npts - 1;
    zin[nb] = a.z[q];
    znext[nb] = a.z[q + 1 < npts ? q + 1 : q];
#pragma unroll
    for (int c = 0; c < 3; ++c) { oin[nb][c] = a.rays_o[ray_of[nb] * 3 + c]; din[nb][c] = a.rays_d[ray_of[nb] * 3 + c]; }
  }
  for (; tile < n_tiles; tile += gridDim.x) {
    st.more = tile + gridDim.x < n_tiles;
    float x[LP][3];
    uint32_t pt_cur[LP], ray_cur[LP];
#pragma unroll
    for (int nb = 0; nb < LP; ++nb) {
      pt_cur[nb] = pt[nb];
      ray_cur[nb] = ray_of[nb];
#pragma unroll
      for (int c = 0; c < 3; ++c) x[nb][c] = add_rn(oin[nb][c], mul_rn(din[nb][c], zin[nb]));
    }
    auto ray_table = [&](const float* (&rb)[LP], int half_table) {
#pragma unroll
      for (int nb = 0; nb < LP; ++nb) {
        uint32_t r = ray_cur[nb];
        asm volatile("" : "+v"(r));
        rb[nb] = a.ray_bias + (size_t)r * ray_bias_floats(W) + half_table * (ray_bias_floats(W) / 2);
      }
    };
    const float* const norb[LP] = {};
    F hid[NB][HC];
#ifdef DFN_TIMING
    {
      const unsigned long long c0 = __builtin_amdgcn_s_memtime();
      float keep = 0.f;
      for (int nb = 0; nb < LP; ++nb) keep += x[nb][0] + x[nb][1] + x[nb][2];
      asm volatile("" ::"v"(keep));
      t_pro += __builtin_amdgcn_s_memtime() - c0;
    }
#endif
    constexpr bool CY = PIPE && P::kSlotsPerChunk == 8, MERGE = UMB >= 8;
    f32x16 carry[NB];
    [[maybe_unused]] uint32_t* mwords = nullptr;
    if constexpr (MASKS) mwords = a.masks + (size_t(tile) * WAVES + st.wave) * (kBwdMaskWords * 64) + st.lane;
    auto sign128 = [&](int l, F (&h)[HC]) {
      if constexpr (MASKS) {
        uint32_t m[2];
        relu_mask<P, HC>(h, m);
        mwords[(2 * l) * 64] = m[0];
        mwords[(2 * l + 1) * 64] = m[1];
      }
    };
    auto sign64 = [&](int word, F (&h)[QC]) {
      if constexpr (MASKS) {
        uint32_t m[1];
        relu_mask<P, QC>(h, m);
        mwords[word * 64] = m[0];
      }
    };
    if constexpr (MASKS) trunk<P, UMB, PIPE, FAST, NB, W>(st, smem, x, hid, carry, sign128);
    else trunk<P, UMB, PIPE, FAST, NB, W>(st, smem, x, hid, carry);
    f32x16 head[NB];
#ifdef DFN_MLP_FOLD_TU
    static_assert(P::kM16 && !MASKS && W == kWidth, "the folded tail exists for the split-f16 16x16x32 render kernel");
    F (&fin)[NB][HC] = hid;
    {
      F dummy[NB][chunks_of<P>(16)];
      layer<P, UMB, PIPE, NB, HC, 0, false, true, false, true, (CY ? 6 : -1), true, false>(st, smem, hid, dummy, head, norb, carry);
    }
#else
    F fin[NB][HC];
    layer<P, UMB, PIPE, NB, HC, MBW, false, true, false, true, (CY ? 6 : -1), true, false>(st, smem, hid, fin, head, norb, carry);
#endif
    sign128(7, hid[0]);
    float o[NB][9];
#pragma unroll
    for (int nb = 0; nb < NB; ++nb) o[nb][3] = head_softplus<P, FAST>(head[nb][0]);
    {
      F de[NB][QC], dummy[NB][chunks_of<P>(16)];
      const float* rb_dir[LP];
      ray_table(rb_dir, 0);
      layer<P, UMB, PIPE, NB, HC, MBQ, true, false, true, true, -1, true, CY>(st, smem, fin, de, head, rb_dir, carry);
      layer<P, UMB, PIPE, NB, QC, 0, false, true, false, !MERGE, (CY ? 2 : -1), true, false>(st, smem, de, dummy, head, norb, carry);
      sign64(16, de[0]);
#pragma unroll
      for (int nb = 0; nb < NB; ++nb)
#pragma unroll
        for (int c = 0; c < 3; ++c) o[nb][c] = head_sigmoid<P, FAST>(head[nb][c]);
    }
    {
      F t0[NB][QC], t1[NB][QC], dummy[NB][chunks_of<P>(16)];
      const float* rb_tr[LP];
      ray_table(rb_tr, 1);
      layer<P, UMB, PIPE, NB, HC, MBQ, true, false, true, true, -1, true, CY>(st, smem, fin, t0, head, rb_tr, carry);
      if (st.more) {
        const uint32_t base = uint32_t(tile + gridDim.x) * uint32_t(PPT) + st.wave * (NB * 32);
        char* slot = smem + ring_slots<P, W>() * USTRIDE + st.wave * (PF_ROUNDS * 8 * 256);
#pragma unroll
        for (int r = 0; r < PF_ROUNDS; ++r) {
          const uint32_t ptn = base + r * 64 + st.lane;
          const uint32_t q = ptn < npts ? ptn : npts - 1;
          const uint32_t ray = q / uint32_t(a.n_samples);
          lds_dma_b32(a.z + q, slot + (r * 8) * 256);
          lds_dma_b32(a.z + (q + 1 < npts ? q + 1 : q), slot + (r * 8 + 7) * 256);
#pragma unroll
          for (int c = 0; c < 3; ++c) {
            lds_dma_b32(a.rays_o + ray * 3 + c, slot + (r * 8 + 1 + c) * 256);
            lds_dma_b32(a.rays_d + ray * 3 + c, slot + (r * 8 + 4 + c) * 256);
          }
        }
      }
      layer<P, UMB, PIPE, NB, QC, MBQ, true, false, false, !MERGE, (CY ? 2 : -1), true, CY>(st, smem, t0, t1, head, norb, carry);
      sign64(17, t0[0]);
      layer<P, UMB, PIPE, NB, QC, MBQ, true, false, false, !MERGE, (CY ? 2 : -1), true, CY>(st, smem, t1, t0, head, norb, carry);
      sign64(18, t1[0]);
      layer<P, UMB, PIPE, NB, QC, MBQ, true, false, false, !MERGE, (CY ? 2 : -1), true, CY>(st, smem, t0, t1, head, norb, carry);
      sign64(19, t0[0]);
      layer<P, UMB, PIPE, NB, QC, 0, false, true, false, !MERGE, (CY ? 2 : -1), true, false>(st, smem, t1, dummy, head, norb, carry);
      sign64(20, t1[0]);
#pragma unroll
      for (int nb = 0; nb < NB; ++nb) {
#pragma unroll
        for (int c = 0; c < 3; ++c) o[nb][4 + c] = head_sigmoid<P, FAST>(head[nb][c]);
        o[nb][7] = head_softplus<P, FAST>(head[nb][3]);
        o[nb][8] = head_softplus<P, FAST>(head[nb][4]);
      }
    }
    uint32_t pt_own[NB], ray_own[NB];
    float z_own[NB], zn_own[NB];
#pragma unroll
    for (int nb = 0; nb < NB; ++nb) {
      if constexpr (P::kM16) {
        const bool n1 = (st.lane & 16) != 0;
        pt_own[nb] = n1 ? pt_cur[1] : pt_cur[0];
        ray_own[nb] = n1 ? ray_cur[1] : ray_cur[0];
        z_own[nb] = n1 ? zin[1] : zin[0];
        zn_own[nb] = n1 ? znext[1] : znext[0];
      } else {
        pt_own[nb] = pt_cur[nb]; ray_own[nb] = ray_cur[nb]; z_own[nb] = zin[nb]; zn_own[nb] = znext[nb];
      }
    }
    if (a.partial) {
      const bool live = h == 0;
      float Pj = 1.f, Ps = 1.f;
      float s_rgb[3] = {0.f, 0.f, 0.f}, s_acc = 0.f, s_dso = 0.f, s_dj = 0.f, s_beta = 0.f;
      [[maybe_unused]] float s_rs[3] = {0.f, 0.f, 0.f}, s_rt[3] = {0.f, 0.f, 0.f};
#pragma unroll
      for (int nb = 0; nb < NB; ++nb) {
        const uint32_t smp = pt_own[nb] - ray_own[nb] * uint32_t(a.n_samples);
        const float delta = smp + 1 == uint32_t(a.n_samples) ? 1e2f : sub_rn(zn_own[nb], z_own[nb]);
        const float sg_s = o[nb][3], sg_t = o[nb][7];
        const float as = live ? sub_rn(1.f, head_exp<P, FAST>(-mul_rn(delta, sg_s))) : 0.f;
        const float at = live ? sub_rn(1.f, head_exp<P, FAST>(-mul_rn(delta, sg_t))) : 0.f;
        const float aj = live ? sub_rn(1.f, head_exp<P, FAST>(-mul_rn(delta, add_rn(sg_s, sg_t)))) : 0.f;
        const float ij = scan32_prod(1.f - aj), is = scan32_prod(1.f - as);
        const float ej = lane_shr1(ij, 1.f), es = lane_shr1(is, 1.f);
        const float Tj = Pj * ej, Ts = Ps * es;
        const float ws = as * Tj, wt = at * Tj, wj = aj * Tj;
#pragma unroll
        for (int c = 0; c < 3; ++c) s_rgb[c] += live ? ws * o[nb][c] + wt * o[nb][4 + c] : 0.f;
        s_acc += wj;
        s_dso += as * Ts * z_own[nb];
        s_dj += wj * z_own[nb];
        s_beta += live ? wt * o[nb][8] : 0.f;
        if constexpr (MAPS) {
          float wt_m = wt;
          asm volatile("" : "+v"(wt_m));
          const float wso = as * Ts;
#pragma unroll
          for (int c = 0; c < 3; ++c) {
            s_rs[c] += live ? wso * o[nb][c] : 0.f;
            s_rt[c] += live ? wt_m * o[nb][4 + c] : 0.f;
          }
        }
        Pj *= read_lane31(ij);
        Ps *= read_lane31(is);
      }
#pragma unroll
      for (int c = 0; c < 3; ++c) s_rgb[c] = read_lane31(scan32_sum(s_rgb[c]));
      s_acc = read_lane31(scan32_sum(s_acc)); s_dso = read_lane31(scan32_sum(s_dso));
      s_dj = read_lane31(scan32_sum(s_dj)); s_beta = read_lane31(scan32_sum(s_beta));
      if constexpr (MAPS) {
#pragma unroll
        for (int c = 0; c < 3; ++c) { s_rs[c] = read_lane31(scan32_sum(s_rs[c])); s_rt[c] = read_lane31(scan32_sum(s_rt[c])); }
      }
      if (st.lane == 0 && pt_own[0] < npts) {
        constexpr int REC = MAPS ? kMapsRecFloats : 12;
        f32x4* dst = reinterpret_cast<f32x4*>(a.partial + (size_t)(pt_own[0] / uint32_t(NB * 32)) * REC);
        dst[0] = f32x4{s_rgb[0], s_rgb[1], s_rgb[2], s_acc};
        dst[1] = f32x4{s_dso, s_dj, s_beta, Pj};
        if constexpr (MAPS) {
          dst[2] = f32x4{Ps, s_rs[0], s_rs[1], s_rs[2]};
          dst[3] = f32x4{s_rt[0], s_rt[1], s_rt[2], 0.f};
        } else {
          dst[2] = f32x4{Ps, 0.f, 0.f, 0.f};
        }
      }
    } else {
#pragma unroll
      for (int nb = 0; nb < NB; ++nb)
        if (h == 0 && pt_own[nb] < npts) {
          float* dst = a.out + (size_t)pt_own[nb] * 9;
#pragma unroll
          for (int c = 0; c < 9; ++c) dst[c] = o[nb][c];
        }
    }
    if (st.more) {
      __builtin_amdgcn_s_waitcnt(0x0F70);
      asm volatile("" ::: "memory");
      tile_coords(tile + gridDim.x);
      const char* slot = smem + ring_slots<P, W>() * USTRIDE + st.wave * (PF_ROUNDS * 8 * 256);
#pragma unroll
      for (int nb = 0; nb < LP; ++nb) {
        int loc = P::kM16 ? 16 * nb + (st.lane & 15) : nb * 32 + p;
        asm volatile("" : "+v"(loc));
        const int r = loc >> 6, l = loc & 63;
        const float* f = reinterpret_cast<const float*>(slot + r * 8 * 256) + l;
        zin[nb] = f[0];
        znext[nb] = f[7 * 64];
#pragma unroll
        for (int c = 0; c < 3; ++c) { oin[nb][c] = f[(1 + c) * 64]; din[nb][c] = f[(4 + c) * 64]; }
      }
    }
  }
  range_report<P>(st.rmax, a.status);
#ifdef DFN_TIMING
  if (a.timing && st.lane == 0) {
    unsigned long long* t = a.timing + (blockIdx.x * WAVES + st.wave) * 4;
    t[0] = __builtin_amdgcn_s_memtime() - t_begin;
    t[1] = st.t_wait;
    t[2] = st.t_sync;
    t[3] = t_pro;
  }
#endif
}

#ifdef DFN_MLP_FOLD_TU
hipError_t launch_mlp_fold(bool maps, const MlpArgs& a, int n_cu, hipStream_t stream) {
  using P = PrecX3M16;
  constexpr int WAVES = 8, UMB = unit_mb<P>(0), NB = 1, PPT = WAVES * NB * 32;
  const long long n_pts = (long long)a.n_rays * a.n_samples;
  if (n_pts <= 0) return hipSuccess;
  if (n_pts >= (1LL << 31)) return hipErrorInvalidValue;
  if (a.masks || (maps && !a.partial)) return hipErrorInvalidValue;
  const long long n_tiles = (n_pts + PPT - 1) / PPT;
  const int grid = int(n_tiles < n_cu ? n_tiles : n_cu);
  const uint32_t lds = lds_bytes<P, UMB, WAVES, NB>();
  void (*kern)(MlpArgs) = maps ? nerfh_fine_fold_kernel<P, false, WAVES, UMB, NB, true, kWidth, false, true>
                               : nerfh_fine_fold_kernel<P, false, WAVES, UMB, NB, true>;
  static bool attr_done[2] = {false, false};
  if (!attr_done[maps]) {
    hipError_t e = hipFuncSetAttribute(reinterpret_cast<const void*>(kern), hipFuncAttributeMaxDynamicSharedMemorySize, int(lds));
    if (e != hipSuccess) return e;
    attr_done[maps] = true;
  }
  MlpArgs b = a;
  if (b.dma_waves == 0) {
    static int env = -1;
    if (env < 0) { const char* e = getenv("DFN_DMA_WAVES"); env = e ? atoi(e) : 0; }
    b.dma_waves = env > 0 ? env : 4;
  }
  hipLaunchKernelGGL(kern, dim3(grid), dim3(WAVES * 64), lds, stream, b);
  return hipGetLastError();
}
#else
template <class P, bool FAST, int WAVES, int UMB, int NB, int WG_PER_CU, bool PIPE, int W = kWidth>
static hipError_t launch_one(bool fine, const MlpArgs& a, int n_cu, hipStream_t stream) {
  constexpr int PPT = WAVES * NB * 32;
  const long long n_pts = (long long)a.n_rays * a.n_samples;
  if (n_pts <= 0) return hipSuccess;
  if (n_pts >= (1LL << 31)) return hipErrorInvalidValue;
  const long long n_tiles = (n_pts + PPT - 1) / PPT;
  const long long slots = (long long)n_cu * WG_PER_CU;
  const int grid = int(n_tiles < slots ? n_tiles : slots);
  const uint32_t lds = lds_bytes<P, UMB, WAVES, NB, W>();
  void (*kern)(MlpArgs) = nullptr;
  int slot = fine ? 1 : 0;
  if constexpr (kMapsTU) {
    if constexpr (W == kWidth && NB <= 2) {
      if (!fine || !a.partial || a.masks) return hipErrorInvalidValue;
      kern = nerfh_fine_kernel<P, FAST, WAVES, UMB, NB, PIPE, W, false, true>;
    } else {
      return hipErrorInvalidValue;
    }
  } else {
    kern = fine ? nerfh_fine_kernel<P, FAST, WAVES, UMB, NB, PIPE, W> : nerfh_coarse_kernel<P, FAST, WAVES, UMB, NB, PIPE, W>;
    if constexpr (P::kSplit && !P::kM16 && NB == 1 && WAVES == 8 && W == kWidth && PIPE) {
      if (fine && a.masks) { kern = nerfh_fine_kernel<P, FAST, WAVES, UMB, NB, PIPE, W, true>; slot = 2; }
    } else if (a.masks) return hipErrorInvalidValue;
  }
  static bool attr_done[3] = {false, false, false};
  if (!attr_done[slot]) {
    hipError_t e = hipFuncSetAttribute(reinterpret_cast<const void*>(kern),
                                       hipFuncAttributeMaxDynamicSharedMemorySize, int(lds));
    if (e != hipSuccess) return e;
    attr_done[slot] = true;
  }
  MlpArgs b = a;
  if (b.dma_waves == 0) {
    static int env = -1;
    if (env < 0) { const char* e = getenv("DFN_DMA_WAVES"); env = e ? atoi(e) : 0; }
    b.dma_waves = env > 0 ? env : (WAVES == 8 ? 4 : WAVES);
  }
  hipLaunchKernelGGL(kern, dim3(grid), dim3(WAVES * 64), lds, stream, b);
  return hipGetLastError();
}

hipError_t DFN_LAUNCH_MLP(bool fine, int prec, int variant, const MlpArgs& a, int n_cu, hipStream_t stream, int width) {
  if (width == 256) {
    if (prec == 0) {
      return launch_one<PrecF16, true, 8, unit_mb_w256<PrecF16>(), 1, 1, false, 256>(fine, a, n_cu, stream);
    }
    if (prec == 2) return launch_one<PrecX3, false, 4, unit_mb_w256<PrecX3>(), 1, 1, false, 256>(fine, a, n_cu, stream);
    return launch_one<PrecF32, false, 4, unit_mb_w256<PrecF32>(), 1, 1, false, 256>(fine, a, n_cu, stream);
  }
  if (width != kWidth) return hipErrorInvalidValue;
  if (variant == 4 && prec != 2) variant = 0;
  if (prec == 0) {
    if (variant == 0) return launch_one<PrecF16, true, 8, 8, 2, 1, true>(fine, a, n_cu, stream);
    if (variant == 1) return launch_one<PrecF16, true, 4, 2, 2, 1, true>(fine, a, n_cu, stream);
    if (variant == 2) return launch_one<PrecF16, true, 4, 8, 3, 1, true>(fine, a, n_cu, stream);
    return launch_one<PrecF16, true, 8, 8, 2, 1, false>(fine, a, n_cu, stream);
  }
  if (prec == 2) {
    if (variant == 3) return launch_one<PrecX3, false, 8, unit_mb<PrecX3>(0), 1, 1, false>(fine, a, n_cu, stream);
    if (variant == 4) return launch_one<PrecX3M16, false, 8, unit_mb<PrecX3M16>(0), 1, 1, true>(fine, a, n_cu, stream);
    return launch_one<PrecX3, false, 8, unit_mb<PrecX3>(0), 1, 1, true>(fine, a, n_cu, stream);
  }
  if (variant == 1) return launch_one<PrecF32, false, 4, 1, 1, 1, false>(fine, a, n_cu, stream);
  return launch_one<PrecF32, false, 8, 1, 1, 1, false>(fine, a, n_cu, stream);
}
#endif

}
```

### dfnet_amd/csrc/nerfh_mlp_core.h

```cpp
#pragma once
#include <hip/hip_runtime.h>
#include <stdint.h>

#include "mfma_frag.h"
#include "nerfh_device.h"
#include "nerfh_kernels.h"
#include "nerfh_layout.h"

#ifndef DFN_PF
#define DFN_PF 3
#endif

namespace dfn {

template <class P> constexpr int chunks_of(int slots) { return slots / P::kSlotsPerChunk; }
template <class P> constexpr int lane_pts(int NB) { return P::kM16 ? 2 : NB; }
template <class P> DFN_HD constexpr int x3_chunk(int i) { return P::kM16 ? (i >> 1) & 1 : i >> 2; }
template <class P> DFN_HD constexpr int x3_pos(int i) { return P::kM16 ? 4 * (i >> 2) + 2 * (i & 1) : 2 * (i & 3); }

template <class P, int KC>
DFN_DEV void set_slot(typename FragOf<P>::type (&arr)[KC], int s, float v) {
  if constexpr (P::kSplit) {
    _Float16 hi, lo;
    x3_split(v, hi, lo);
    arr[s >> 3].hi[s & 7] = hi;
    arr[s >> 3].lo[s & 7] = lo;
  } else if constexpr (P::kSlotsPerChunk == 8) arr[s >> 3][s & 7] = (_Float16)v;
  else arr[s] = v;
}

struct Stager {
  const char* blob;
  const uint32_t* tab;
  int n_units;
  int u;
  uint32_t slot;
  uint32_t ring;
  uint32_t ustride;
  int lane, wave, waves;
  int dma_waves;
  uint32_t ubase, uoff;
  uint32_t pf_off, pf_size;
  unsigned long long t_sync, t_wait, t_last;
  unsigned long long* trace;
  int n_trace;
  bool more;
  float in_scale, out_scale;
  float lane_mul;
  uint32_t rmax;
};

DFN_DEV uint32_t pk_max_u16(uint32_t a, uint32_t b) {
  uint32_t r;
  asm("v_pk_max_u16 %0, %1, %2" : "=v"(r) : "v"(a), "v"(b));
  return r;
}
DFN_DEV void range_track(uint32_t& rmax, uint32_t packed, bool nonneg) {
  rmax = pk_max_u16(rmax, nonneg ? packed : (packed & 0x7fff7fffu));
}
template <class P>
DFN_DEV void range_report(uint32_t rmax, int* status) {
  if constexpr (P::kSlotsPerChunk == 8) {
    const uint32_t thr = P::kSplit ? 0x7bffu : 0x7c00u;
    if (status && ((rmax & 0xffffu) >= thr || (rmax >> 16) >= thr)) atomicOr(status, P::kSplit ? 2 : 1);
  }
}

DFN_DEV void lds_dma_b128(const void* gptr, const char* lds_dst) {
  const uint32_t off = (uint32_t)(size_t)DFN_LDS_PTR(lds_dst);
  asm volatile("s_mov_b32 m0, %1\n\tglobal_load_lds_dwordx4 %0, off" ::"v"(gptr), "s"(off) : "memory");
}
DFN_DEV void lds_dma_b32(const void* gptr, const char* lds_dst) {
  const uint32_t off = (uint32_t)(size_t)DFN_LDS_PTR(lds_dst);
  asm volatile("s_mov_b32 m0, %1\n\tglobal_load_lds_dword %0, off" ::"v"(gptr), "s"(off) : "memory");
}

DFN_DEV void stage_issue_at(const Stager& st, char* smem, uint32_t off, uint32_t size, uint32_t lds_off) {
  const char* src = st.blob + off + st.lane * 16;
  if (st.wave >= st.dma_waves) return;
  for (uint32_t p = st.wave * kPiece; p < size; p += st.dma_waves * kPiece) lds_dma_b128(src + p, smem + lds_off + p);
}
typedef const uint32_t __attribute__((address_space(4))) const_u32;
DFN_DEV uint32_t tab_entry(const Stager& st, int i) {
  return reinterpret_cast<const_u32*>(reinterpret_cast<uint64_t>(st.tab))[i];
}
DFN_DEV void stage_issue(const Stager& st, char* smem, int unit, uint32_t lds_off) {
  stage_issue_at(st, smem, tab_entry(st, 2 * unit), tab_entry(st, 2 * unit + 1), lds_off);
}

DFN_DEV void stage_prime(Stager& st, char* smem, uint32_t unit_stride, uint32_t ring = 3) {
  st.slot = 0; st.ring = ring; st.ustride = unit_stride;
  st.u = 0;
  stage_issue(st, smem, 0, 0);
  stage_issue(st, smem, st.n_units > 1 ? 1 : 0, unit_stride);
  const int n2 = st.n_units > 2 ? 2 : 0;
  st.pf_off = tab_entry(st, 2 * n2);
  st.pf_size = tab_entry(st, 2 * n2 + 1);
  __builtin_amdgcn_s_waitcnt(0x0F70);
  asm volatile("" ::: "memory");
  __syncthreads();
}

DFN_DEV uint32_t open_unit(Stager& st) {
  const uint32_t cur = st.slot * st.ustride;
  st.slot = st.slot + 1 == st.ring ? 0u : st.slot + 1;
  int nxt = st.u + 1;
  if (nxt == st.n_units) nxt = 0;
  st.u = nxt;
  return cur;
}

DFN_DEV void mid_sync(Stager& st, char* smem) {
#ifdef DFN_TIMING
  const unsigned long long c0 = __builtin_amdgcn_s_memtime();
#endif
  __builtin_amdgcn_s_waitcnt(0x0F70);
  asm volatile("" ::: "memory");
#ifdef DFN_TIMING
  const unsigned long long c1 = __builtin_amdgcn_s_memtime();
#endif
  int n2 = st.u + 1;
  bool next_tile = st.u == 0;
  if (n2 >= st.n_units) { n2 -= st.n_units; next_tile = true; }
  const uint32_t dst = (st.slot + 1 == st.ring ? 0u : st.slot + 1) * st.ustride;
  __builtin_amdgcn_s_barrier();
  asm volatile("" ::: "memory");
#ifdef DFN_TIMING
  const unsigned long long c2 = __builtin_amdgcn_s_memtime();
  st.t_wait += c1 - c0;
  st.t_sync += c2 - c1;
  if (st.trace && st.n_trace < 96 && st.lane == 0) {
    st.trace[2 * st.n_trace] = c0;
    st.trace[2 * st.n_trace + 1] = c2;
  }
  ++st.n_trace;
#endif
  if (!next_tile || st.more) stage_issue_at(st, smem, st.pf_off, st.pf_size, dst);
  {
    int n3 = n2 + 1;
    if (n3 >= st.n_units) n3 -= st.n_units;
    st.pf_off = tab_entry(st, 2 * n3);
    st.pf_size = tab_entry(st, 2 * n3 + 1);
  }
}

template <class P>
DFN_DEV typename FragOf<P>::type load_afrag(const char* p);

template <class P, int NB, int KC>
DFN_DEV void mblock_mma(const char* smem, uint32_t wb, const typename FragOf<P>::type (&Bin)[NB][KC],
                        f32x16 (&acc)[NB]) {
  using F = typename FragOf<P>::type;
#pragma unroll
  for (int kc = 0; kc < KC; ++kc) {
    const F a = load_afrag<P>(smem + wb + kc * 64 * P::kLaneBytes);
#pragma unroll
    for (int nb = 0; nb < NB; ++nb) acc[nb] = mfma<P>(a, Bin[nb][kc], acc[nb]);
  }
}

template <class P>
DFN_DEV typename FragOf<P>::type load_afrag(const char* p) {
  if constexpr (P::kSplit) {
    half8x2 f;
    f.hi = *reinterpret_cast<const half8*>(p);
    f.lo = *reinterpret_cast<const half8*>(p + 1024);
    return f;
  } else {
    return *reinterpret_cast<const typename FragOf<P>::type*>(p);
  }
}

DFN_DEV f32x16 load16(const float* p) {
  const f32x4* q = reinterpret_cast<const f32x4*>(p);
  f32x4 a = q[0], b = q[1], c = q[2], d = q[3];
  f32x16 r;
#pragma unroll
  for (int i = 0; i < 4; ++i) { r[i] = a[i]; r[4 + i] = b[i]; r[8 + i] = c[i]; r[12 + i] = d[i]; }
  return r;
}
DFN_DEV f32x16 load_bias_m16(const float* p) {
  const f32x4* q = reinterpret_cast<const f32x4*>(p);
  const f32x4 a = q[0], b = q[1];
  f32x16 r = {};
#pragma unroll
  for (int i = 0; i < 4; ++i) { r[i] = a[i]; r[4 + i] = b[i]; }
  return r;
}
DFN_DEV f32x16 load_raybias_m16(const float* const (&rb)[2], int mb, int g) {
  f32x16 r;
#pragma unroll
  for (int nb = 0; nb < 2; ++nb) {
    const f32x4* q = reinterpret_cast<const f32x4*>(rb[nb] + mb * 32 + (g & 1) * 16 + 4 * (g >> 1));
    const f32x4 a = q[0], b = q[2];
#pragma unroll
    for (int i = 0; i < 4; ++i) { r[4 * nb + i] = a[i]; r[8 + 4 * nb + i] = b[i]; }
  }
  return r;
}
DFN_DEV f32x4 sub4(const f32x16& v, int o) { return f32x4{v[o], v[o + 1], v[o + 2], v[o + 3]}; }
DFN_DEV void put4(f32x16& v, int o, const f32x4& x) { v[o] = x[0]; v[o + 1] = x[1]; v[o + 2] = x[2]; v[o + 3] = x[3]; }

template <class P, bool RELU, int OC>
DFN_DEV void store_hidden(const f32x16& acc, typename FragOf<P>::type (&out)[OC], int mb, float oscale, uint32_t& rmax) {
  if constexpr (P::kSplit) {
    typedef __fp16 pk2 __attribute__((ext_vector_type(2)));
    const float os = oscale * kX3ActScale;
#pragma unroll
    for (int c = 0; c < 2; ++c)
#pragma unroll
      for (int j = 0; j < 8; j += 2) {
        float x0 = acc[8 * c + j] * os, x1 = acc[8 * c + j + 1] * os;
        if (RELU) { x0 = fmaxf(x0, 0.f); x1 = fmaxf(x1, 0.f); }
        const pk2 h = __builtin_amdgcn_cvt_pkrtz(x0, x1);
        const uint32_t hb = __builtin_bit_cast(uint32_t, h);
        float r0, r1;
        asm("v_fma_mix_f32 %0, %1, -1.0, %2 op_sel_hi:[1,0,0]" : "=v"(r0) : "v"(hb), "v"(x0));
        asm("v_fma_mix_f32 %0, %1, -1.0, %2 op_sel:[1,0,0] op_sel_hi:[1,0,0]" : "=v"(r1) : "v"(hb), "v"(x1));
        const pk2 l = __builtin_amdgcn_cvt_pkrtz(r0, r1);
        range_track(rmax, hb, RELU);
        const int oc = 2 * mb + x3_chunk<P>(4 * c + j / 2), oj = x3_pos<P>(4 * c + j / 2);
        out[oc].hi[oj] = (_Float16)h[0]; out[oc].hi[oj + 1] = (_Float16)h[1];
        out[oc].lo[oj] = (_Float16)l[0]; out[oc].lo[oj + 1] = (_Float16)l[1];
      }
  } else if constexpr (P::kSlotsPerChunk == 8) {
#pragma unroll
    for (int c = 0; c < 2; ++c) {
      half8 v;
#pragma unroll
      for (int j = 0; j < 8; ++j) v[j] = (_Float16)acc[8 * c + j];
      if (RELU) {
        const half8 zero = {0, 0, 0, 0, 0, 0, 0, 0};
        v = __builtin_elementwise_max(v, zero);
      }
      {
        typedef uint32_t u32x4 __attribute__((ext_vector_type(4)));
        u32x4 w = __builtin_bit_cast(u32x4, v);
        if (!RELU) w &= 0x7fff7fffu;
        rmax = pk_max_u16(rmax, pk_max_u16(pk_max_u16(w[0], w[1]), pk_max_u16(w[2], w[3])));
      }
      out[2 * mb + c] = v;
    }
  } else {
#pragma unroll
    for (int r = 0; r < 16; ++r) out[16 * mb + r] = RELU ? fmaxf(acc[r], 0.f) : acc[r];
  }
}

template <class P, bool RELU, int OC>
DFN_DEV void store_hidden(const f32x16& acc, typename FragOf<P>::type (&out)[OC], int mb, float oscale = 1.f) {
  uint32_t unused = 0;
  store_hidden<P, RELU>(acc, out, mb, oscale, unused);
}

template <class P, bool RELU, int OC>
DFN_DEV void store_hidden_piece(const f32x16& acc, typename FragOf<P>::type (&out)[OC], int mb, int i, float oscale, uint32_t& rmax) {
  if constexpr (P::kSplit) {
    typedef _Float16 half2v __attribute__((ext_vector_type(2)));
    const int c = i >> 2, j = (i & 3) * 2;
    uint32_t hb, lb;
    float t0, t1;
    if (RELU)
      asm volatile("v_mul_f32 %2, %4, %6\n\tv_mul_f32 %3, %5, %6\n\tv_max_f32 %2, %2, 0\n\tv_max_f32 %3, %3, 0\n\t"
                   "v_cvt_pkrtz_f16_f32 %0, %2, %3\n\t"
                   "v_fma_mix_f32 %2, %0, -1.0, %2 op_sel_hi:[1,0,0]\n\t"
                   "v_fma_mix_f32 %3, %0, -1.0, %3 op_sel:[1,0,0] op_sel_hi:[1,0,0]\n\t"
                   "v_cvt_pkrtz_f16_f32 %1, %2, %3"
                   : "=&v"(hb), "=&v"(lb), "=&v"(t0), "=&v"(t1) : "v"(acc[8 * c + j]), "v"(acc[8 * c + j + 1]), "v"(oscale));
    else
      asm volatile("v_mul_f32 %2, %4, %6\n\tv_mul_f32 %3, %5, %6\n\t"
                   "v_cvt_pkrtz_f16_f32 %0, %2, %3\n\t"
                   "v_fma_mix_f32 %2, %0, -1.0, %2 op_sel_hi:[1,0,0]\n\t"
                   "v_fma_mix_f32 %3, %0, -1.0, %3 op_sel:[1,0,0] op_sel_hi:[1,0,0]\n\t"
                   "v_cvt_pkrtz_f16_f32 %1, %2, %3"
                   : "=&v"(hb), "=&v"(lb), "=&v"(t0), "=&v"(t1) : "v"(acc[8 * c + j]), "v"(acc[8 * c + j + 1]), "v"(oscale));
    if (RELU) asm volatile("v_pk_max_u16 %0, %0, %1" : "+v"(rmax) : "v"(hb));
    else range_track(rmax, hb, false);
    const half2v hv = __builtin_bit_cast(half2v, hb), lv = __builtin_bit_cast(half2v, lb);
    const int oc = 2 * mb + x3_chunk<P>(i), oj = x3_pos<P>(i);
    out[oc].hi[oj] = hv[0]; out[oc].hi[oj + 1] = hv[1];
    out[oc].lo[oj] = lv[0]; out[oc].lo[oj + 1] = lv[1];
  } else if constexpr (P::kSlotsPerChunk == 8) {
    typedef _Float16 half2v __attribute__((ext_vector_type(2)));
    const int c = i >> 2, j = i & 3;
    uint32_t bits;
    if (RELU)
      asm volatile("v_cvt_pk_f16_f32 %0, %1, %2\n\tv_pk_max_f16 %0, %0, 0" : "=v"(bits) : "v"(acc[8 * c + 2 * j]), "v"(acc[8 * c + 2 * j + 1]));
    else
      asm volatile("v_cvt_pk_f16_f32 %0, %1, %2" : "=v"(bits) : "v"(acc[8 * c + 2 * j]), "v"(acc[8 * c + 2 * j + 1]));
    if (RELU) asm volatile("v_pk_max_u16 %0, %0, %1" : "+v"(rmax) : "v"(bits));
    else range_track(rmax, bits, false);
    const half2v v = __builtin_bit_cast(half2v, bits);
    out[2 * mb + c][2 * j] = v[0];
    out[2 * mb + c][2 * j + 1] = v[1];
  } else {
    float x0 = acc[2 * i], x1 = acc[2 * i + 1];
    asm volatile("" : "+v"(x0), "+v"(x1));
    x0 = RELU ? fmaxf(x0, 0.f) : x0;
    x1 = RELU ? fmaxf(x1, 0.f) : x1;
    asm volatile("" : "+v"(x0), "+v"(x1));
    out[16 * mb + 2 * i] = x0;
    out[16 * mb + 2 * i + 1] = x1;
  }
}

struct X3Piece {
  uint32_t hb, hs, lb;
  float t0, t1;
  template <bool RELU>
  DFN_DEV void A(const f32x16& acc, int i) {
    const int c = i >> 2, j = (i & 3) * 2;
    if (RELU) asm volatile("v_max_f32 %0, %2, 0\n\tv_max_f32 %1, %3, 0" : "=&v"(t0), "=&v"(t1) : "v"(acc[8 * c + j]), "v"(acc[8 * c + j + 1]));
    else asm volatile("v_mov_b32 %0, %2\n\tv_mov_b32 %1, %3" : "=&v"(t0), "=&v"(t1) : "v"(acc[8 * c + j]), "v"(acc[8 * c + j + 1]));
  }
  DFN_DEV void B(float s, uint32_t s2) {
    asm volatile("v_cvt_pkrtz_f16_f32 %0, %2, %3\n\t"
                 "v_pk_mul_f16 %1, %0, %5\n\t"
                 "v_fma_mix_f32 %2, %2, %4, -%1 op_sel_hi:[0,0,1]\n\t"
                 "v_fma_mix_f32 %3, %3, %4, -%1 op_sel:[0,0,1] op_sel_hi:[0,0,1]"
                 : "=&v"(hb), "=&v"(hs), "+v"(t0), "+v"(t1) : "v"(s), "v"(s2));
  }
  DFN_DEV void B1(uint32_t s2) {
    asm volatile("v_cvt_pkrtz_f16_f32 %0, %2, %3\n\t"
                 "v_pk_mul_f16 %1, %0, %4"
                 : "=&v"(hb), "=&v"(hs) : "v"(t0), "v"(t1), "v"(s2));
  }
  DFN_DEV void B2(float s) {
    asm volatile("v_fma_mix_f32 %0, %0, %2, -%3 op_sel_hi:[0,0,1]\n\t"
                 "v_fma_mix_f32 %1, %1, %2, -%3 op_sel:[0,0,1] op_sel_hi:[0,0,1]"
                 : "+v"(t0), "+v"(t1) : "v"(s), "v"(hs));
  }
  template <bool RELU, class P = PrecX3, int OC>
  DFN_DEV void C(half8x2 (&out)[OC], int mb, int i, uint32_t& rmax) {
    typedef _Float16 half2v __attribute__((ext_vector_type(2)));
    const int c = x3_chunk<P>(i), j = x3_pos<P>(i);
    asm volatile("v_cvt_pkrtz_f16_f32 %0, %1, %2" : "=v"(lb) : "v"(t0), "v"(t1));
    if (RELU) asm volatile("v_pk_max_u16 %0, %0, %1" : "+v"(rmax) : "v"(hb));
    else range_track(rmax, hb, false);
    const half2v hv = __builtin_bit_cast(half2v, hs), lv = __builtin_bit_cast(half2v, lb);
    out[2 * mb + c].hi[j] = hv[0]; out[2 * mb + c].hi[j + 1] = hv[1];
    out[2 * mb + c].lo[j] = lv[0]; out[2 * mb + c].lo[j + 1] = lv[1];
  }
};

template <class P, int UMB, bool PIPE, int NB, int KC, int MB, bool RELU, bool EXTRA, bool RAYBIAS, bool NEWUNIT,
          int CIN, bool CIN_RELU, bool COUT, bool NOBIAS = false, bool SCALE_FIRST = false, bool TRACK = true>
DFN_DEV void layer(Stager& st, char* smem, typename FragOf<P>::type (&Bin)[NB][KC],
                   typename FragOf<P>::type (&Bout)[NB][(MB ? MB : 1) * chunks_of<P>(16)],
                   f32x16 (&head)[NB], const float* const (&raybias)[lane_pts<P>(NB)], f32x16 (&carry)[NB]) {
  using F = typename FragOf<P>::type;
  static_assert(!P::kM16 || (PIPE && NB == 1 && !SCALE_FIRST), "the 16x16x32 split-f16 layer is the pipelined one-point-block form");
  constexpr int TOT = MB + (EXTRA ? 1 : 0);
  constexpr int PF = P::kSplit ? 2 : (P::kSlotsPerChunk == 8 ? DFN_PF : 4);
  constexpr uint32_t FB = 64 * P::kLaneBytes;
  constexpr int PPK = (8 * NB + KC - 1) / KC;
  constexpr int PPKI = CIN > 0 ? (8 * NB + CIN - 1) / CIN : 0;
  static_assert(CIN < 0 || (PIPE && P::kSlotsPerChunk == 8 && CIN > 0 && CIN + 1 < KC + 1), "carry-in needs the pipelined f16 path");
  static_assert(!COUT || (PIPE && MB >= 1 && !EXTRA), "carry-out needs a regular last M-block");
  static_assert(NEWUNIT || UMB >= TOT, "a layer that continues a unit must fit in it");
  const int h = st.lane >> 5, g16 = st.lane >> 4;
  uint32_t rmax_sink = 0;
  uint32_t& rmax_ = TRACK ? st.rmax : rmax_sink;
  const float pscale = P::kSplit ? st.out_scale * st.lane_mul * kX3ActScale : 1.f;
  uint32_t pscale2 = 0;
  if constexpr (P::kSplit) asm("v_cvt_pkrtz_f16_f32 %0, %1, %1" : "=v"(pscale2) : "v"(pscale));
  constexpr bool RB_ALL = RAYBIAS && NB <= 2;
  f32x16 rb[RB_ALL ? TOT : 1][NB];
  if (RB_ALL) {
#pragma unroll
    for (int mb = 0; mb < TOT; ++mb)
#pragma unroll
      for (int nb = 0; nb < NB; ++nb) {
        if constexpr (P::kM16) rb[mb][nb] = load_raybias_m16(raybias, mb, g16);
        else rb[mb][nb] = load16(raybias[nb] + (mb * 2 + h) * 16);
        if constexpr (P::kSplit) rb[mb][nb] *= st.in_scale;
      }
  }
  f32x16 pend[PIPE ? NB : 1];
#pragma unroll
  for (int u0 = 0; u0 < TOT; u0 += UMB) {
    const int nmb = (TOT - u0) < UMB ? (TOT - u0) : UMB;
    const int nt = nmb * KC;
    uint32_t ub;
    if (NEWUNIT) { ub = open_unit(st); st.ubase = ub; st.uoff = 0; }
    else ub = st.ubase + st.uoff;
    st.uoff += nmb * KC * FB + nmb * 128;
    const char* wl = smem + ub + st.lane * (P::kSplit ? 16 : P::kLaneBytes);
    const char* bl = smem + ub + nmb * KC * FB + (P::kM16 ? g16 * 32 : h * 64);
    F a[PF];
#define DFN_AFRAG(t) load_afrag<P>(wl + (t) * FB)
#pragma unroll
    for (int t = 0; t < PF; ++t)
      if (t < nt) a[t] = DFN_AFRAG(t);
    f32x16 bias = {};
    auto load_bias = [&](const char* p) {
      if constexpr (P::kM16) return load_bias_m16(reinterpret_cast<const float*>(p));
      else return load16(reinterpret_cast<const float*>(p));
    };
    if (!RAYBIAS && !NOBIAS) bias = load_bias(bl);
#pragma unroll
    for (int lm = 0; lm < UMB; ++lm) {
      if (lm < nmb) {
        const int mb = u0 + lm;
        f32x16 acc[NB];
        f32x16 bias_next = bias;
        if (RAYBIAS) {
#pragma unroll
          for (int nb = 0; nb < NB; ++nb) {
            if constexpr (P::kM16) acc[nb] = RB_ALL ? rb[RB_ALL ? mb : 0][nb] : load_raybias_m16(raybias, mb, g16);
            else acc[nb] = RB_ALL ? rb[RB_ALL ? mb : 0][nb] : load16(raybias[nb] + (mb * 2 + h) * 16);
            if constexpr (P::kSplit && !RB_ALL) acc[nb] *= st.in_scale;
          }
        }
#pragma unroll
        for (int kc = 0; kc < KC; ++kc) {
          const int t = lm * KC + kc;
          if (NEWUNIT && lm == 0 && kc == (KC > 1 ? KC / 2 : 0)) mid_sync(st, smem);
          const F cur = a[t % PF];
          if (t + PF < nt) a[t % PF] = DFN_AFRAG(t + PF);
          if (kc == (PIPE ? KC / 2 : 0) && !RAYBIAS && !NOBIAS && lm + 1 < nmb) bias_next = load_bias(bl + (lm + 1) * 128);
          __builtin_amdgcn_sched_barrier(0);
          if constexpr (P::kSplit && PIPE && NB == 1 && !SCALE_FIRST) {
            constexpr int PPKI_ = (CIN > 0) ? (8 * NB + CIN - 1) / CIN : 1, PPK_ = (8 * NB + KC - 1) / KC;
            constexpr int NPMAX = PPKI_ > PPK_ ? PPKI_ : PPK_;
            const bool from_carry = CIN > 0 && mb == 0 && kc < CIN, from_pend = mb >= 1;
            const int np = from_carry ? PPKI_ : (from_pend ? PPK_ : 0), base = kc * np;
            X3Piece pc[NPMAX];
            const bool late = kc == 0;
#define DFN_X3_PARTS_A \
            _Pragma("unroll") for (int q = 0; q < NPMAX; ++q) \
              if (q < np && base + q < 8) { \
                if (from_carry) pc[q].template A<CIN_RELU>(carry[0], base + q); \
                else pc[q].template A<RELU>(pend[0], base + q); \
              }
#define DFN_X3_PARTS_B \
            _Pragma("unroll") for (int q = 0; q < NPMAX; ++q) \
              if (q < np && base + q < 8) pc[q].B(pscale, pscale2);
            if constexpr (P::kM16) {
              const int ms = kc & 1, bc = 2 * (kc >> 1);
              f32x4 c0, c1;
              if (kc < 2 && !RAYBIAS) { c0 = sub4(bias, 4 * ms); c1 = c0; }
              else { c0 = sub4(acc[0], 8 * ms); c1 = sub4(acc[0], 8 * ms + 4); }
#define DFN_X3_PARTS(...) \
              _Pragma("unroll") for (int q = 0; q < NPMAX; ++q) \
                if (q < np && base + q < 8) { __VA_ARGS__; }
              c0 = __builtin_amdgcn_mfma_f32_16x16x32_f16(cur.hi, Bin[0][bc].hi, c0, 0, 0, 0);
              c1 = __builtin_amdgcn_mfma_f32_16x16x32_f16(cur.hi, Bin[0][bc + 1].hi, c1, 0, 0, 0);
              __builtin_amdgcn_sched_barrier(0);
              DFN_X3_PARTS_A
              __builtin_amdgcn_sched_barrier(0);
              c0 = __builtin_amdgcn_mfma_f32_16x16x32_f16(cur.hi, Bin[0][bc].lo, c0, 0, 0, 0);
              __builtin_amdgcn_sched_barrier(0);
              DFN_X3_PARTS(pc[q].B1(pscale2))
              __builtin_amdgcn_sched_barrier(0);
              c1 = __builtin_amdgcn_mfma_f32_16x16x32_f16(cur.hi, Bin[0][bc + 1].lo, c1, 0, 0, 0);
              __builtin_amdgcn_sched_barrier(0);
              DFN_X3_PARTS(pc[q].B2(pscale))
              __builtin_amdgcn_sched_barrier(0);
              c0 = __builtin_amdgcn_mfma_f32_16x16x32_f16(cur.lo, Bin[0][bc].hi, c0, 0, 0, 0);
              __builtin_amdgcn_sched_barrier(0);
              DFN_X3_PARTS(if (from_carry) pc[q].template C<CIN_RELU, P>(Bin[0], CIN / 2, base + q, rmax_);
                           else pc[q].template C<RELU, P>(Bout[0], mb - 1, base + q, rmax_))
              __builtin_amdgcn_sched_barrier(0);
              c1 = __builtin_amdgcn_mfma_f32_16x16x32_f16(cur.lo, Bin[0][bc + 1].hi, c1, 0, 0, 0);
#undef DFN_X3_PARTS
              put4(acc[0], 8 * ms, c0);
              put4(acc[0], 8 * ms + 4, c1);
              if (from_carry && kc == CIN - 1) asm volatile("s_nop 3");
              __builtin_amdgcn_sched_barrier(0);
              continue;
            }
            f32x16 c0 = (kc == 0) ? (RAYBIAS ? acc[0] : bias) : acc[0];
            c0 = __builtin_amdgcn_mfma_f32_32x32x16_f16(cur.hi, Bin[0][kc].hi, c0, 0, 0, 0);
            __builtin_amdgcn_sched_barrier(0);
            if (!late) { DFN_X3_PARTS_A }
            __builtin_amdgcn_sched_barrier(0);
            c0 = __builtin_amdgcn_mfma_f32_32x32x16_f16(cur.hi, Bin[0][kc].lo, c0, 0, 0, 0);
            __builtin_amdgcn_sched_barrier(0);
            if (!late) { DFN_X3_PARTS_B }
            __builtin_amdgcn_sched_barrier(0);
            c0 = __builtin_amdgcn_mfma_f32_32x32x16_f16(cur.lo, Bin[0][kc].hi, c0, 0, 0, 0);
            __builtin_amdgcn_sched_barrier(0);
            if (late) { DFN_X3_PARTS_A DFN_X3_PARTS_B }
#undef DFN_X3_PARTS_A
#undef DFN_X3_PARTS_B
#pragma unroll
            for (int q = 0; q < NPMAX; ++q)
              if (q < np && base + q < 8) {
                if (from_carry) pc[q].template C<CIN_RELU>(Bin[0], CIN / 2, base + q, rmax_);
                else pc[q].template C<RELU>(Bout[0], mb - 1, base + q, rmax_);
              }
            acc[0] = c0;
            if (from_carry && kc == CIN - 1) asm volatile("s_nop 3");
            __builtin_amdgcn_sched_barrier(0);
            continue;
          }
          if constexpr (!P::kM16) {
#pragma unroll
          for (int nb = 0; nb < NB; ++nb) {
            if (kc == 0) acc[nb] = mfma<P>(cur, Bin[nb][0], RAYBIAS ? acc[nb] : bias);
            else acc[nb] = mfma<P>(cur, Bin[nb][kc], acc[nb]);
          }
          }
          if (CIN > 0 && mb == 0 && kc < CIN) {
#pragma unroll
            for (int q = 0; q < PPKI; ++q) {
              const int piece = kc * PPKI + q;
              if (piece < 8 * NB) store_hidden_piece<P, CIN_RELU>(carry[piece >> 3], Bin[piece >> 3], CIN / 2, piece & 7, pscale, rmax_);
            }
            if (kc == CIN - 1) asm volatile("s_nop 3");
          }
          if (PIPE && mb >= 1) {
#pragma unroll
            for (int q = 0; q < PPK; ++q) {
              const int piece = kc * PPK + q;
              if (piece < 8 * NB) store_hidden_piece<P, RELU>(pend[piece >> 3], Bout[piece >> 3], mb - 1, piece & 7, pscale, rmax_);
            }
          }
          __builtin_amdgcn_sched_barrier(0);
        }
        bias = bias_next;
        if (mb < MB) {
          if (PIPE) {
#pragma unroll
            for (int nb = 0; nb < NB; ++nb) pend[nb] = acc[nb];
          } else {
#pragma unroll
            for (int nb = 0; nb < NB; ++nb) store_hidden<P, RELU>(acc[nb], Bout[nb], mb, st.out_scale * st.lane_mul, rmax_);
          }
        } else {
#pragma unroll
          for (int nb = 0; nb < NB; ++nb) {
            head[nb] = acc[nb];
            if constexpr (P::kSplit) head[nb] *= st.out_scale * st.lane_mul;
            if constexpr (P::kM16) {
              const f32x16 v = head[nb];
              const bool g1 = (g16 & 1) != 0;
#pragma unroll
              for (int c = 0; c < 8; ++c) head[nb][c] = g1 ? v[8 * (c >> 2) + 4 + (c & 3)] : v[8 * (c >> 2) + (c & 3)];
            }
          }
        }
      }
    }
  }
  if (PIPE && MB >= 1 && !EXTRA) {
    if (COUT) {
#pragma unroll
      for (int nb = 0; nb < NB; ++nb) carry[nb] = pend[nb];
    } else {
#pragma unroll
      for (int nb = 0; nb < NB; ++nb) store_hidden<P, RELU>(pend[nb], Bout[nb], MB - 1, st.out_scale * st.lane_mul, rmax_);
    }
  }
}

template <class P, bool FAST, int NB, int PC>
DFN_DEV void posenc_xyz(const float (&x)[NB][3], int h, typename FragOf<P>::type (&pe)[NB][PC]) {
  const float base = h ? 32.f : 1.f;
#pragma unroll
  for (int nb = 0; nb < NB; ++nb) {
#pragma unroll
    for (int c = 0; c < 3; ++c) {
      const float xc = x[nb][c];
      if (FAST) {
        float uh, ul, sn[5], cs[5];
        rev_split(xc, uh, ul);
        rev_sincos_octaves5(uh, ul, base, sn, cs);
#pragma unroll
        for (int k = 0; k < 5; ++k) {
          set_slot<P>(pe[nb], 6 * k + c, sn[k]);
          set_slot<P>(pe[nb], 6 * k + 3 + c, cs[k]);
        }
      } else if constexpr (P::kSplit) {
        float uh, ul;
        rev_split(xc, uh, ul);
#pragma unroll
        for (int k = 0; k < 5; ++k) {
          float sn, cs;
          rev_sincos(uh, ul, base * float(1 << k), sn, cs);
          set_slot<P>(pe[nb], 6 * k + c, sn);
          set_slot<P>(pe[nb], 6 * k + 3 + c, cs);
        }
      } else {
        const float xb = xc * base;
#pragma unroll
        for (int k = 0; k < 5; ++k) {
          const float a = xb * float(1 << k);
          set_slot<P>(pe[nb], 6 * k + c, sinf(a));
          set_slot<P>(pe[nb], 6 * k + 3 + c, cosf(a));
        }
      }
    }
    set_slot<P>(pe[nb], 30, h ? x[nb][2] : x[nb][0]);
    set_slot<P>(pe[nb], 31, h ? 0.f : x[nb][1]);
  }
}

template <class P, int PC>
DFN_DEV void posenc_xyz_m16(const float (&x)[2][3], int g, typename FragOf<P>::type (&pe)[1][PC]) {
  static_assert(P::kM16 && PC == 4, "16 slots of two points");
  auto put = [&](int n, int s, float v) {
    _Float16 hi, lo;
    x3_split(v, hi, lo);
    pe[0][2 * (s >> 3) + n].hi[s & 7] = hi;
    pe[0][2 * (s >> 3) + n].lo[s & 7] = lo;
  };
  const float base = float(1 << (2 * g));
  const float f6 = g == 2 ? 512.f : 256.f, f7 = g == 0 ? 256.f : 512.f;
#pragma unroll
  for (int n = 0; n < 2; ++n) {
    float uh[3], ul[3];
#pragma unroll
    for (int c = 0; c < 3; ++c) rev_split(x[n][c], uh[c], ul[c]);
#pragma unroll
    for (int k = 0; k < 2; ++k)
#pragma unroll
      for (int c = 0; c < 3; ++c) {
        float sn, cs;
        rev_sincos(uh[c], ul[c], base * float(1 << k), sn, cs);
        put(n, 6 * k + c, sn);
        put(n, 6 * k + 3 + c, cs);
      }
    float s6, c6, s7, c7;
    rev_sincos(g == 0 ? uh[0] : (g == 1 ? uh[2] : uh[1]), g == 0 ? ul[0] : (g == 1 ? ul[2] : ul[1]), f6, s6, c6);
    rev_sincos(g == 0 ? uh[1] : (g == 1 ? uh[0] : uh[2]), g == 0 ? ul[1] : (g == 1 ? ul[0] : ul[2]), f7, s7, c7);
    if (g == 3) { s6 = x[n][0]; c6 = x[n][1]; s7 = x[n][2]; c7 = 0.f; }
    put(n, 12, s6); put(n, 13, c6); put(n, 14, s7); put(n, 15, c7);
  }
}

struct NoTrunkHook {
  template <class A> DFN_DEV void operator()(int, A&) const {}
};
template <class P, int UMB, bool PIPE, bool FAST, int NB, int W = kWidth, class Hook = NoTrunkHook>
DFN_DEV void trunk(Stager& st, char* smem, const float (&x)[lane_pts<P>(NB)][3],
                   typename FragOf<P>::type (&out)[NB][chunks_of<P>(W / 2)], f32x16 (&carry)[NB], Hook hook = Hook()) {
  using F = typename FragOf<P>::type;
  constexpr int PC = chunks_of<P>(32), HC = chunks_of<P>(W / 2), MBW = W / 32;
  constexpr bool CY = PIPE && P::kSlotsPerChunk == 8;
  constexpr int CI = CY ? HC - 2 : -1;
  static_assert(!PIPE || W == kWidth, "the pipelined epilogue is tuned for netwidth 128");
  const int h = st.lane >> 5;
  f32x16 nohead[NB];
  const float* const norb[lane_pts<P>(NB)] = {};
  F pe[NB][PC];
  auto encode = [&](const float (&xx)[lane_pts<P>(NB)][3]) {
    if constexpr (P::kM16) { static_assert(!FAST, "split-f16 only"); posenc_xyz_m16<P, PC>(xx, st.lane >> 4, pe); }
    else posenc_xyz<P, FAST, NB, PC>(xx, h, pe);
  };
  encode(x);
  F a[NB][HC], b[NB][HC];
  layer<P, UMB, PIPE, NB, PC, MBW, true, false, false, true, -1, true, CY>(st, smem, pe, a, nohead, norb, carry);
  layer<P, UMB, PIPE, NB, HC, MBW, true, false, false, true, CI, true, CY>(st, smem, a, b, nohead, norb, carry);
  hook(0, a[0]);
  layer<P, UMB, PIPE, NB, HC, MBW, true, false, false, true, CI, true, CY>(st, smem, b, a, nohead, norb, carry);
  hook(1, b[0]);
  layer<P, UMB, PIPE, NB, HC, MBW, true, false, false, true, CI, true, CY>(st, smem, a, b, nohead, norb, carry);
  hook(2, a[0]);
  {
    F cat[NB][PC + HC];
    if constexpr (P::kSlotsPerChunk == 8 && (!PIPE || P::kSplit)) {
      float x2[lane_pts<P>(NB)][3];
#pragma unroll
      for (int nb = 0; nb < lane_pts<P>(NB); ++nb)
#pragma unroll
        for (int c = 0; c < 3; ++c) {
          x2[nb][c] = x[nb][c];
          asm volatile("" : "+v"(x2[nb][c]));
        }
      encode(x2);
    }
#pragma unroll
    for (int nb = 0; nb < NB; ++nb) {
#pragma unroll
      for (int i = 0; i < PC; ++i) cat[nb][i] = pe[nb][i];
#pragma unroll
      for (int i = 0; i < HC; ++i) cat[nb][PC + i] = b[nb][i];
    }
    layer<P, l5_unit_mb_p<P>(UMB), PIPE, NB, PC + HC, MBW, true, false, false, true, (CY ? PC + HC - 2 : -1), true, CY>(st, smem, cat, a, nohead, norb, carry);
    hook(3, reinterpret_cast<F(&)[HC]>(cat[0][PC]));
  }
  layer<P, UMB, PIPE, NB, HC, MBW, true, false, false, true, CI, true, CY>(st, smem, a, b, nohead, norb, carry);
  hook(4, a[0]);
  layer<P, UMB, PIPE, NB, HC, MBW, true, false, false, true, CI, true, CY>(st, smem, b, a, nohead, norb, carry);
  hook(5, b[0]);
  layer<P, UMB, PIPE, NB, HC, MBW, true, false, false, true, CI, true, CY>(st, smem, a, out, nohead, norb, carry);
  hook(6, a[0]);
}

}
```

Before: 5.465 million rays/s.

## Add half-height M16 head blocks that skip the unused second M-subblock

Adds a new default MLP variant whose sigma/rgb/transient head layers are packed at half height: only the first 16-row M-subblock of the m16 head blocks is stored and computed, since the heads have at most four outputs. The layer template gains a HALF mode that halves K-chunk iteration, zero-inits accumulators and handles the carried-in tail block specially. The fine kernel also drops the beta (transient uncertainty) softplus and accumulation when maps are not requested. This reduces MFMA work and weight staging for head layers, at the cost of another kernel instantiation, a separate packed net for the maps path, and subtle scheduling changes.

Result: faster. 5.559 million rays/s (median of 6 runs) (+1.7%).

```diff
diff --git a/dfnet_amd/csrc/nerfh_api.hip b/dfnet_amd/csrc/nerfh_api.hip
--- a/dfnet_amd/csrc/nerfh_api.hip
+++ b/dfnet_amd/csrc/nerfh_api.hip
@@ -105,10 +105,10 @@
         if (n.tab) (void)hipFree(n.tab);
         n = PackedNet();
       }
-  for (auto& n : h->bwd) {
-    if (n.blob) (void)hipFree(n.blob);
-    if (n.tab) (void)hipFree(n.tab);
-    n = PackedNet();
+  for (PackedNet* n : {&h->bwd[0], &h->bwd[1], &h->bwd[2], &h->half_maps}) {
+    if (n->blob) (void)hipFree(n->blob);
+    if (n->tab) (void)hipFree(n->tab);
+    *n = PackedNet();
   }
   if (h->extra) (void)hipFree(h->extra);
   h->extra = nullptr;
@@ -157,6 +157,8 @@
   int width() const { return h->desc.width; }
   mutable int fwd_units = 0;
   std::vector<float> fold_dir, fold_tr;
+  bool half_heads = false, half_thead = false;
+  bool half_block(int layer) const { return half_heads && (layer == LY_SIG || layer == LY_RGB || (layer == LY_THEAD && half_thead)); }
   Mat mat(const std::string& key) const {
     Mat m;
     const auto& w = h->params.at(pre + key + ".weight");
@@ -221,7 +223,9 @@
     const LayerShape sh = layer_shape(layer, width());
     const int KC = sh.slots / P::kSlotsPerChunk;
     Elem* frag = reinterpret_cast<Elem*>(base);
-    float* bias = reinterpret_cast<float*>(base + size_t(group) * KC * 64 * P::kLaneBytes);
+    const bool half = P::kM16 && half_block(layer);
+    const int KCP = half ? KC / 2 : KC;
+    float* bias = reinterpret_cast<float*>(base + size_t(group) * KCP * 64 * P::kLaneBytes);
     for (int g = 0; g < group; ++g) {
       const int mb = mb0 + g;
       if constexpr (P::kM16) {
@@ -233,13 +237,14 @@
         };
         for (int lane = 0; lane < 64; ++lane)
           for (int kc = 0; kc < KC; ++kc) {
+            if (half && (kc & 1)) continue;
             Mat m;
             int row;
             source(16 * (kc & 1) + (lane & 15), m, row);
             for (int j = 0; j < 8; ++j) {
               const int col = col_source_m16(layer, lane >> 4, 8 * (kc >> 1) + j);
               const float v = (row >= 0 && col >= 0 && col < m.cols) ? m.w[size_t(row) * m.cols + col] : 0.f;
-              Elem* fr = frag + (size_t(g) * KC + kc) * 64 * 16;
+              Elem* fr = frag + (size_t(g) * KCP + (half ? kc >> 1 : kc)) * 64 * 16;
               const Elem hi = Elem(v * wscale);
               fr[lane * 8 + j] = hi;
               fr[512 + lane * 8 + j] = Elem(v * wscale - float(hi));
@@ -369,7 +374,8 @@
   template <class P>
   uint32_t blocks_bytes(int layer, int group) const {
     const LayerShape sh = layer_shape(layer, width());
-    return uint32_t(group) * (sh.slots / P::kSlotsPerChunk) * 64 * P::kLaneBytes + uint32_t(group) * 128;
+    const bool half = P::kM16 && half_block(layer);
+    return uint32_t(group) * (sh.slots / P::kSlotsPerChunk / (half ? 2 : 1)) * 64 * P::kLaneBytes + uint32_t(group) * 128;
   }
 
   template <class P>
@@ -413,7 +419,7 @@
       const int lu = (seq[li] == LY_L5 && l5_umb > 0) ? l5_umb : umb;
       for (int mb0 = 0; mb0 < sh.mb; mb0 += lu) {
         const int group = sh.mb - mb0 < lu ? sh.mb - mb0 : lu;
-        const uint32_t bytes = unit_bytes<P>(sh.slots, group);
+        const uint32_t bytes = unit_bytes<P>(sh.slots, group, P::kM16 && half_block(seq[li]));
         const uint32_t off = uint32_t(blob.size());
         blob.resize(off + bytes, 0);
         tab.push_back(off);
@@ -555,9 +561,13 @@
   for (int f = 0; f < 2; ++f)
     for (int prec = 0; prec < 3; ++prec)
       for (int var = 0; var < kVariants; ++var) {
-        const bool fold = var == kFoldVariant;
-        if (fold && !(f == 1 && prec == DFN_PREC_F16X3)) continue;
+        const bool half = var == kHalfVariant;
+        const bool fold = var == kFoldVariant || (half && f == 1);
+        if (var == kFoldVariant && !(f == 1 && prec == DFN_PREC_F16X3)) continue;
+        if (half && prec != DFN_PREC_F16X3) continue;
         Packer pk{h, f ? "fine." : "coarse."};
+        pk.half_heads = half;
+        pk.half_thead = half;
         std::vector<uint8_t> blob;
         std::vector<uint32_t> tab;
         PackedNet& n = h->net[f][prec][var];
@@ -579,7 +589,20 @@
             fold_final(h->params.at("fine.dir_encoding.0.weight"), Wd / 2, ldd, F, bF, Wd, pk.fold_dir, fold_bd);
             fold_final(h->params.at("fine.transient_encoding.0.weight"), Wd / 2, ldt, F, bF, Wd, pk.fold_tr, fold_bt);
             pk.pack<PrecX3M16>(f, unit_mb<PrecX3M16>(var), false, blob, tab, l5_unit_mb_p<PrecX3M16>(unit_mb<PrecX3M16>(var)), true);
-          } else if (var == 4) pk.pack<PrecX3M16>(f, unit_mb<PrecX3M16>(var), false, blob, tab, l5_unit_mb_p<PrecX3M16>(unit_mb<PrecX3M16>(var)));
+            if (half) {
+              std::vector<uint8_t> mblob;
+              std::vector<uint32_t> mtab;
+              pk.half_thead = false;
+              pk.pack<PrecX3M16>(f, unit_mb<PrecX3M16>(var), false, mblob, mtab, l5_unit_mb_p<PrecX3M16>(unit_mb<PrecX3M16>(var)), true);
+              PackedNet& m = h->half_maps;
+              m.in_scale = n.in_scale;
+              int rc = upload(mblob.data(), mblob.size(), reinterpret_cast<void**>(&m.blob));
+              if (rc) return rc;
+              rc = upload(mtab.data(), mtab.size() * 4, reinterpret_cast<void**>(&m.tab));
+              if (rc) return rc;
+              m.n_units = int(mtab.size() / 2);
+            }
+          } else if (var == 4 || half) pk.pack<PrecX3M16>(f, unit_mb<PrecX3M16>(var), false, blob, tab, l5_unit_mb_p<PrecX3M16>(unit_mb<PrecX3M16>(var)));
           else pk.pack<PrecX3>(f, unit_mb<PrecX3>(var), false, blob, tab, l5_unit_mb_p<PrecX3>(unit_mb<PrecX3>(var)));
         }
         int rc = upload(blob.data(), blob.size(), reinterpret_cast<void**>(&n.blob));
@@ -730,18 +753,20 @@
   return DFN_OK;
 }
 
+constexpr int kDefaultVariant = kHalfVariant;
 static int mlp_variant_128();
 static int mlp_variant_of(dfn_nerfh_t h) { return h->desc.width == kWidth ? mlp_variant_128() : 0; }
 static int mlp_variant_128() {
   static int v = -1;
   if (v < 0) {
     const char* e = getenv("DFN_MLP_VARIANT");
-    v = (e && e[0] >= '0' && e[0] < '0' + kVariants) ? e[0] - '0' : kFoldVariant;
+    v = (e && e[0] >= '0' && e[0] < '0' + kVariants) ? e[0] - '0' : kDefaultVariant;
   }
   return v;
 }
-static int base_variant(int var) { return var == kFoldVariant ? 4 : var; }
-static bool fold_fine(int var, int prec) { return var == kFoldVariant && prec == DFN_PREC_F16X3; }
+static int base_variant(int var) { return var == kFoldVariant || var == kHalfVariant ? 4 : var; }
+static bool fold_fine(int var, int prec) { return (var == kFoldVariant || var == kHalfVariant) && prec == DFN_PREC_F16X3; }
+static bool half_heads(int var, int prec) { return var == kHalfVariant && prec == DFN_PREC_F16X3; }
 
 static int* range_flag_of(dfn_nerfh_t h) { return h->range_flag; }
 
@@ -767,13 +792,15 @@
   if (int rc = check_net(h, prec, "dfn_mlp_coarse", true)) return rc;
   if (!n_rays) return DFN_OK;
   if (!rays_o || !rays_d || !sigma || Nc < 1) return set_error(DFN_ERR_ARG, "dfn_mlp_coarse: bad argument");
+  const bool half = half_heads(mlp_variant_of(h), prec);
   const int var = base_variant(mlp_variant_of(h));
-  const PackedNet& n = h->net[0][prec][var];
+  const PackedNet& n = h->net[0][prec][half ? kHalfVariant : var];
   MlpArgs a{n.blob, n.tab, n.n_units, rays_o, rays_d, nullptr, nullptr, sigma, nullptr, (long long)n_rays, Nc, near, far, nullptr, n.in_scale,
             h->render_flags & DFN_RENDER_LINDISP};
   a.status = range_flag_of(h);
   ScopedTimer t(0, HS(stream));
-  CHECK_HIP(launch_mlp(false, prec, var, a, device_cu_count(), HS(stream), h->desc.width), "dfn_mlp_coarse");
+  if (half) CHECK_HIP(launch_mlp_half(false, false, a, device_cu_count(), HS(stream)), "dfn_mlp_coarse");
+  else CHECK_HIP(launch_mlp(false, prec, var, a, device_cu_count(), HS(stream), h->desc.width), "dfn_mlp_coarse");
   return DFN_OK;
 }
 
@@ -927,8 +954,9 @@
   const int seg = prec == DFN_PREC_F16 ? 64 : 32;
   const bool fused = !raw_out && Nf % seg == 0 && !(prec == DFN_PREC_F16 && var == 2) && h->desc.width == kWidth;
   const int cprec = (h->render_flags & DFN_RENDER_COARSE_F16) ? DFN_PREC_F16 : prec;
-  const PackedNet& nc = h->net[0][cprec][var];
-  const PackedNet& nf = h->net[1][prec][fold ? kFoldVariant : var];
+  const bool half_c = half_heads(mlp_variant_of(h), cprec), half_f = half_heads(mlp_variant_of(h), prec) && fused;
+  const PackedNet& nc = h->net[0][cprec][half_c ? kHalfVariant : var];
+  const PackedNet& nf = half_f ? (want_maps ? h->half_maps : h->net[1][prec][kHalfVariant]) : h->net[1][prec][fold ? kFoldVariant : var];
   const int cus = device_cu_count();
   const size_t chunk = chunk_rays(n_rays);
   for (size_t r0 = 0; r0 < n_rays; r0 += chunk) {
@@ -943,7 +971,8 @@
                  h->render_flags & DFN_RENDER_LINDISP};
       a.status = range_flag_of(h);
       ScopedTimer t(0, s);
-      CHECK_HIP(launch_mlp(false, cprec, var, a, cus, s, h->desc.width), "render: coarse MLP");
+      if (half_c) CHECK_HIP(launch_mlp_half(false, false, a, cus, s), "render: coarse MLP (half-height heads)");
+      else CHECK_HIP(launch_mlp(false, cprec, var, a, cus, s, h->desc.width), "render: coarse MLP");
     }
     {
       ScopedTimer t(DFN_PROF_SAMPLE_FINE, s);
@@ -958,7 +987,8 @@
       MlpArgs a{nf.blob, nf.tab, nf.n_units, co, cd, w.z, w.bias, raw, fused ? w.partial : nullptr, (long long)n, Nf, 0.f, 0.f, g_timing_buf, nf.in_scale};
       a.status = range_flag_of(h);
       ScopedTimer t(1, s);
-      if (fold) CHECK_HIP(launch_mlp_fold(fused && want_maps, a, cus, s), "render: fine MLP (folded)");
+      if (half_f) CHECK_HIP(launch_mlp_half(true, want_maps, a, cus, s), "render: fine MLP (half-height heads)");
+      else if (fold) CHECK_HIP(launch_mlp_fold(fused && want_maps, a, cus, s), "render: fine MLP (folded)");
       else if (fused && want_maps) CHECK_HIP(launch_mlp_maps(true, prec, var, a, cus, s, h->desc.width), "render: fine MLP (maps)");
       else CHECK_HIP(launch_mlp(true, prec, var, a, cus, s, h->desc.width), "render: fine MLP");
     }
diff --git a/dfnet_amd/csrc/nerfh_handle.h b/dfnet_amd/csrc/nerfh_handle.h
--- a/dfnet_amd/csrc/nerfh_handle.h
+++ b/dfnet_amd/csrc/nerfh_handle.h
@@ -20,6 +20,7 @@
   std::map<std::string, std::vector<float>> params;
   bool committed = false;
   PackedNet net[2][3][dfn::kVariants];
+  PackedNet half_maps;
   PackedNet bwd[3];
   float* extra = nullptr;
   dfn::RayBiasWeights rb{};
diff --git a/dfnet_amd/csrc/nerfh_kernels.h b/dfnet_amd/csrc/nerfh_kernels.h
--- a/dfnet_amd/csrc/nerfh_kernels.h
+++ b/dfnet_amd/csrc/nerfh_kernels.h
@@ -30,6 +30,7 @@
 hipError_t launch_mlp(bool fine, int prec, int variant, const MlpArgs& a, int n_cu, hipStream_t stream, int width = 128);
 hipError_t launch_mlp_maps(bool fine, int prec, int variant, const MlpArgs& a, int n_cu, hipStream_t stream, int width = 128);
 hipError_t launch_mlp_fold(bool maps, const MlpArgs& a, int n_cu, hipStream_t stream);
+hipError_t launch_mlp_half(bool fine, bool maps, const MlpArgs& a, int n_cu, hipStream_t stream);
 
 hipError_t launch_raygen(int H, int W, float focal, const float* c2w, float* rays_o, float* rays_d,
                          float* viewdirs, hipStream_t stream, int frames = 1);
diff --git a/dfnet_amd/csrc/nerfh_layout.h b/dfnet_amd/csrc/nerfh_layout.h
--- a/dfnet_amd/csrc/nerfh_layout.h
+++ b/dfnet_amd/csrc/nerfh_layout.h
@@ -80,8 +80,9 @@
 constexpr float kX3ActScale = 16.f;
 struct PrecX3M16 { static constexpr int kSlotsPerChunk = 8, kLaneBytes = 32; static constexpr bool kSplit = true, kM16 = true; };
 
-constexpr int kVariants = 6;
+constexpr int kVariants = 7;
 constexpr int kFoldVariant = 5;
+constexpr int kHalfVariant = 6;
 template <class P> DFN_HD constexpr int unit_mb(int variant) {
   return P::kSlotsPerChunk == 1 ? 1 : (P::kSplit ? 2 : (variant == 1 ? 2 : 8));
 }
@@ -93,8 +94,8 @@
 DFN_HD constexpr uint32_t align_piece(uint32_t b) { return (b + kPiece - 1) / kPiece * kPiece; }
 
 template <class P>
-DFN_HD constexpr uint32_t unit_bytes(int slots, int nmb) {
-  return align_piece(uint32_t(nmb) * (slots / P::kSlotsPerChunk) * 64 * P::kLaneBytes + uint32_t(nmb) * 2 * 16 * 4);
+DFN_HD constexpr uint32_t unit_bytes(int slots, int nmb, bool half = false) {
+  return align_piece(uint32_t(nmb) * (slots / P::kSlotsPerChunk / (half ? 2 : 1)) * 64 * P::kLaneBytes + uint32_t(nmb) * 2 * 16 * 4);
 }
 DFN_HD constexpr int l5_unit_mb(int umb) { return umb >= 8 ? 2 : umb; }
 template <class P> DFN_HD constexpr int l5_unit_mb_p(int umb) { return (P::kSplit && umb == 2) ? 1 : l5_unit_mb(umb); }
diff --git a/dfnet_amd/csrc/nerfh_mlp.hip b/dfnet_amd/csrc/nerfh_mlp.hip
--- a/dfnet_amd/csrc/nerfh_mlp.hip
+++ b/dfnet_amd/csrc/nerfh_mlp.hip
@@ -19,11 +19,19 @@
 constexpr bool kMapsTU = false;
 #define DFN_LAUNCH_MLP launch_mlp
 #endif
+#ifdef DFN_MLP_HALF_TU
+#define DFN_FINE_KERNEL nerfh_fine_half_kernel
+#define DFN_COARSE_KERNEL nerfh_coarse_half_kernel
+constexpr bool kHalfHeads = true;
+#else
 #ifdef DFN_MLP_FOLD_TU
 #define DFN_FINE_KERNEL nerfh_fine_fold_kernel
 #else
 #define DFN_FINE_KERNEL nerfh_fine_kernel
 #endif
+#define DFN_COARSE_KERNEL nerfh_coarse_kernel
+constexpr bool kHalfHeads = false;
+#endif
 
 template <class P, bool FAST> DFN_DEV float head_softplus(float v) { return FAST ? softplus_fast(v) : (P::kSplit ? softplus_hw(v) : softplus(v)); }
 template <class P, bool FAST> DFN_DEV float head_sigmoid(float v) { return FAST ? sigmoid_fast(v) : (P::kSplit ? sigmoid_hw(v) : sigmoid(v)); }
@@ -40,7 +48,7 @@
 }
 
 template <class P, bool FAST, int WAVES, int UMB, int NB, bool PIPE, int W = kWidth>
-__global__ __launch_bounds__(WAVES * 64, (mlp_min_blocks<P, WAVES, NB, W>())) void nerfh_coarse_kernel(MlpArgs a) {
+__global__ __launch_bounds__(WAVES * 64, (mlp_min_blocks<P, WAVES, NB, W>())) void DFN_COARSE_KERNEL(MlpArgs a) {
   extern __shared__ __attribute__((aligned(16))) char smem[];
   constexpr int PPT = WAVES * NB * 32;
   using F = typename FragOf<P>::type;
@@ -94,7 +102,7 @@
     f32x16 head[NB];
     F dummy[NB][chunks_of<P>(16)];
     const float* const norb[LP] = {};
-    layer<P, UMB, PIPE, NB, chunks_of<P>(W / 2), 0, false, true, false, !MERGE, (CY ? 6 : -1), true, false>(st, smem, hid, dummy, head, norb, carry);
+    layer<P, UMB, PIPE, NB, chunks_of<P>(W / 2), 0, false, true, false, !MERGE, (CY ? 6 : -1), true, false, false, false, true, kHalfHeads>(st, smem, hid, dummy, head, norb, carry);
 #pragma unroll
     for (int nb = 0; nb < NB; ++nb)
       if (h == 0 && pt[nb] < npts) a.out[pt[nb]] = head_softplus<P, FAST>(head[nb][0]);
@@ -113,6 +121,7 @@
   constexpr uint32_t USTRIDE = max_unit_bytes<P>(UMB, W);
   constexpr int PF_ROUNDS = (NB * 32 + 63) / 64;
   constexpr int LP = lane_pts<P>(NB);
+  constexpr bool NOBETA = kHalfHeads && !MAPS;
   using F = typename FragOf<P>::type;
   Stager st;
   st.blob = a.blob; st.tab = a.tab; st.n_units = a.n_units; st.u = 0;
@@ -217,7 +226,7 @@
     F (&fin)[NB][HC] = hid;
     {
       F dummy[NB][chunks_of<P>(16)];
-      layer<P, UMB, PIPE, NB, HC, 0, false, true, false, true, (CY ? 6 : -1), true, false>(st, smem, hid, dummy, head, norb, carry);
+      layer<P, UMB, PIPE, NB, HC, 0, false, true, false, true, (CY ? 6 : -1), true, false, false, false, true, kHalfHeads>(st, smem, hid, dummy, head, norb, carry);
     }
 #else
     F fin[NB][HC];
@@ -232,7 +241,7 @@
       const float* rb_dir[LP];
       ray_table(rb_dir, 0);
       layer<P, UMB, PIPE, NB, HC, MBQ, true, false, true, true, -1, true, CY>(st, smem, fin, de, head, rb_dir, carry);
-      layer<P, UMB, PIPE, NB, QC, 0, false, true, false, !MERGE, (CY ? 2 : -1), true, false>(st, smem, de, dummy, head, norb, carry);
+      layer<P, UMB, PIPE, NB, QC, 0, false, true, false, !MERGE, (CY ? 2 : -1), true, false, false, false, true, kHalfHeads>(st, smem, de, dummy, head, norb, carry);
       sign64(16, de[0]);
 #pragma unroll
       for (int nb = 0; nb < NB; ++nb)
@@ -267,14 +276,15 @@
       sign64(18, t1[0]);
       layer<P, UMB, PIPE, NB, QC, MBQ, true, false, false, !MERGE, (CY ? 2 : -1), true, CY>(st, smem, t0, t1, head, norb, carry);
       sign64(19, t0[0]);
-      layer<P, UMB, PIPE, NB, QC, 0, false, true, false, !MERGE, (CY ? 2 : -1), true, false>(st, smem, t1, dummy, head, norb, carry);
+      layer<P, UMB, PIPE, NB, QC, 0, false, true, false, !MERGE, (CY ? 2 : -1), true, false, false, false, true, NOBETA>(st, smem, t1, dummy, head, norb, carry);
       sign64(20, t1[0]);
 #pragma unroll
       for (int nb = 0; nb < NB; ++nb) {
 #pragma unroll
         for (int c = 0; c < 3; ++c) o[nb][4 + c] = head_sigmoid<P, FAST>(head[nb][c]);
         o[nb][7] = head_softplus<P, FAST>(head[nb][3]);
-        o[nb][8] = head_softplus<P, FAST>(head[nb][4]);
+        if constexpr (NOBETA) o[nb][8] = 0.f;
+        else o[nb][8] = head_softplus<P, FAST>(head[nb][4]);
       }
     }
     uint32_t pt_own[NB], ray_own[NB];
@@ -313,7 +323,7 @@
         s_acc += wj;
         s_dso += as * Ts * z_own[nb];
         s_dj += wj * z_own[nb];
-        s_beta += live ? wt * o[nb][8] : 0.f;
+        if constexpr (!NOBETA) s_beta += live ? wt * o[nb][8] : 0.f;
         if constexpr (MAPS) {
           float wt_m = wt;
           asm volatile("" : "+v"(wt_m));
@@ -330,7 +340,8 @@
 #pragma unroll
       for (int c = 0; c < 3; ++c) s_rgb[c] = read_lane31(scan32_sum(s_rgb[c]));
       s_acc = read_lane31(scan32_sum(s_acc)); s_dso = read_lane31(scan32_sum(s_dso));
-      s_dj = read_lane31(scan32_sum(s_dj)); s_beta = read_lane31(scan32_sum(s_beta));
+      s_dj = read_lane31(scan32_sum(s_dj));
+      if constexpr (!NOBETA) s_beta = read_lane31(scan32_sum(s_beta));
       if constexpr (MAPS) {
 #pragma unroll
         for (int c = 0; c < 3; ++c) { s_rs[c] = read_lane31(scan32_sum(s_rs[c])); s_rt[c] = read_lane31(scan32_sum(s_rt[c])); }
@@ -386,7 +397,37 @@
 #endif
 }
 
-#ifdef DFN_MLP_FOLD_TU
+#if defined(DFN_MLP_HALF_TU)
+hipError_t launch_mlp_half(bool fine, bool maps, const MlpArgs& a, int n_cu, hipStream_t stream) {
+  using P = PrecX3M16;
+  constexpr int WAVES = 8, UMB = unit_mb<P>(0), NB = 1, PPT = WAVES * NB * 32;
+  const long long n_pts = (long long)a.n_rays * a.n_samples;
+  if (n_pts <= 0) return hipSuccess;
+  if (n_pts >= (1LL << 31)) return hipErrorInvalidValue;
+  if (a.masks || (fine && !a.partial) || (maps && !fine)) return hipErrorInvalidValue;
+  const long long n_tiles = (n_pts + PPT - 1) / PPT;
+  const int grid = int(n_tiles < n_cu ? n_tiles : n_cu);
+  const uint32_t lds = lds_bytes<P, UMB, WAVES, NB>();
+  const int slot = fine ? (maps ? 2 : 1) : 0;
+  void (*kern)(MlpArgs) = !fine ? nerfh_coarse_half_kernel<P, false, WAVES, UMB, NB, true>
+                          : maps ? nerfh_fine_half_kernel<P, false, WAVES, UMB, NB, true, kWidth, false, true>
+                                 : nerfh_fine_half_kernel<P, false, WAVES, UMB, NB, true>;
+  static bool attr_done[3] = {false, false, false};
+  if (!attr_done[slot]) {
+    hipError_t e = hipFuncSetAttribute(reinterpret_cast<const void*>(kern), hipFuncAttributeMaxDynamicSharedMemorySize, int(lds));
+    if (e != hipSuccess) return e;
+    attr_done[slot] = true;
+  }
+  MlpArgs b = a;
+  if (b.dma_waves == 0) {
+    static int env = -1;
+    if (env < 0) { const char* e = getenv("DFN_DMA_WAVES"); env = e ? atoi(e) : 0; }
+    b.dma_waves = env > 0 ? env : 4;
+  }
+  hipLaunchKernelGGL(kern, dim3(grid), dim3(WAVES * 64), lds, stream, b);
+  return hipGetLastError();
+}
+#elif defined(DFN_MLP_FOLD_TU)
 hipError_t launch_mlp_fold(bool maps, const MlpArgs& a, int n_cu, hipStream_t stream) {
   using P = PrecX3M16;
   constexpr int WAVES = 8, UMB = unit_mb<P>(0), NB = 1, PPT = WAVES * NB * 32;
diff --git a/dfnet_amd/csrc/nerfh_mlp_core.h b/dfnet_amd/csrc/nerfh_mlp_core.h
--- a/dfnet_amd/csrc/nerfh_mlp_core.h
+++ b/dfnet_amd/csrc/nerfh_mlp_core.h
@@ -344,7 +344,7 @@
 };
 
 template <class P, int UMB, bool PIPE, int NB, int KC, int MB, bool RELU, bool EXTRA, bool RAYBIAS, bool NEWUNIT,
-          int CIN, bool CIN_RELU, bool COUT, bool NOBIAS = false, bool SCALE_FIRST = false, bool TRACK = true>
+          int CIN, bool CIN_RELU, bool COUT, bool NOBIAS = false, bool SCALE_FIRST = false, bool TRACK = true, bool HALF = false>
 DFN_DEV void layer(Stager& st, char* smem, typename FragOf<P>::type (&Bin)[NB][KC],
                    typename FragOf<P>::type (&Bout)[NB][(MB ? MB : 1) * chunks_of<P>(16)],
                    f32x16 (&head)[NB], const float* const (&raybias)[lane_pts<P>(NB)], f32x16 (&carry)[NB]) {
@@ -358,6 +358,11 @@
   static_assert(CIN < 0 || (PIPE && P::kSlotsPerChunk == 8 && CIN > 0 && CIN + 1 < KC + 1), "carry-in needs the pipelined f16 path");
   static_assert(!COUT || (PIPE && MB >= 1 && !EXTRA), "carry-out needs a regular last M-block");
   static_assert(NEWUNIT || UMB >= TOT, "a layer that continues a unit must fit in it");
+  static_assert(!HALF || (P::kM16 && EXTRA && MB == 0 && !RAYBIAS && KC % 2 == 0 && CIN >= 2 && CIN % 2 == 0 && CIN + 2 == KC),
+                "a half-height block is a PrecX3M16 head layer whose last 32-K chunk is the carried-in M-block");
+  constexpr int KCL = HALF ? KC / 2 : KC;
+  constexpr int CINL = HALF ? CIN / 2 : CIN;
+  constexpr bool TAILBLK = HALF && CINL == 1;
   const int h = st.lane >> 5, g16 = st.lane >> 4;
   uint32_t rmax_sink = 0;
   uint32_t& rmax_ = TRACK ? st.rmax : rmax_sink;
@@ -380,13 +385,13 @@
 #pragma unroll
   for (int u0 = 0; u0 < TOT; u0 += UMB) {
     const int nmb = (TOT - u0) < UMB ? (TOT - u0) : UMB;
-    const int nt = nmb * KC;
+    const int nt = nmb * KCL;
     uint32_t ub;
     if (NEWUNIT) { ub = open_unit(st); st.ubase = ub; st.uoff = 0; }
     else ub = st.ubase + st.uoff;
-    st.uoff += nmb * KC * FB + nmb * 128;
+    st.uoff += nmb * KCL * FB + nmb * 128;
     const char* wl = smem + ub + st.lane * (P::kSplit ? 16 : P::kLaneBytes);
-    const char* bl = smem + ub + nmb * KC * FB + (P::kM16 ? g16 * 32 : h * 64);
+    const char* bl = smem + ub + nmb * KCL * FB + (P::kM16 ? g16 * 32 : h * 64);
     F a[PF];
 #define DFN_AFRAG(t) load_afrag<P>(wl + (t) * FB)
 #pragma unroll
@@ -403,6 +408,10 @@
       if (lm < nmb) {
         const int mb = u0 + lm;
         f32x16 acc[NB];
+        if constexpr (HALF) {
+#pragma unroll
+          for (int nb = 0; nb < NB; ++nb) acc[nb] = f32x16{};
+        }
         f32x16 bias_next = bias;
         if (RAYBIAS) {
 #pragma unroll
@@ -413,17 +422,18 @@
           }
         }
 #pragma unroll
-        for (int kc = 0; kc < KC; ++kc) {
-          const int t = lm * KC + kc;
-          if (NEWUNIT && lm == 0 && kc == (KC > 1 ? KC / 2 : 0)) mid_sync(st, smem);
+        for (int kc = 0; kc < KCL; ++kc) {
+          const int t = lm * KCL + kc;
+          if (NEWUNIT && lm == 0 && kc == (KCL > 1 ? KCL / 2 : 0)) mid_sync(st, smem);
           const F cur = a[t % PF];
           if (t + PF < nt) a[t % PF] = DFN_AFRAG(t + PF);
-          if (kc == (PIPE ? KC / 2 : 0) && !RAYBIAS && !NOBIAS && lm + 1 < nmb) bias_next = load_bias(bl + (lm + 1) * 128);
+          if (kc == (PIPE ? KCL / 2 : 0) && !RAYBIAS && !NOBIAS && lm + 1 < nmb) bias_next = load_bias(bl + (lm + 1) * 128);
           __builtin_amdgcn_sched_barrier(0);
           if constexpr (P::kSplit && PIPE && NB == 1 && !SCALE_FIRST) {
-            constexpr int PPKI_ = (CIN > 0) ? (8 * NB + CIN - 1) / CIN : 1, PPK_ = (8 * NB + KC - 1) / KC;
+            constexpr int PPKI_ = TAILBLK ? 4 : ((CIN > 0) ? (8 * NB + CINL - 1) / CINL : 1), PPK_ = (8 * NB + KCL - 1) / KCL;
             constexpr int NPMAX = PPKI_ > PPK_ ? PPKI_ : PPK_;
-            const bool from_carry = CIN > 0 && mb == 0 && kc < CIN, from_pend = mb >= 1;
+            static_assert(!HALF || NPMAX <= 4, "half 1's pieces must not start in the first chunk");
+            const bool from_carry = CIN > 0 && mb == 0 && kc < CINL, from_pend = mb >= 1;
             const int np = from_carry ? PPKI_ : (from_pend ? PPK_ : 0), base = kc * np;
             X3Piece pc[NPMAX];
             const bool late = kc == 0;
@@ -437,9 +447,9 @@
             _Pragma("unroll") for (int q = 0; q < NPMAX; ++q) \
               if (q < np && base + q < 8) pc[q].B(pscale, pscale2);
             if constexpr (P::kM16) {
-              const int ms = kc & 1, bc = 2 * (kc >> 1);
+              const int ms = HALF ? 0 : (kc & 1), bc = HALF ? 2 * kc : 2 * (kc >> 1);
               f32x4 c0, c1;
-              if (kc < 2 && !RAYBIAS) { c0 = sub4(bias, 4 * ms); c1 = c0; }
+              if (kc < (HALF ? 1 : 2) && !RAYBIAS) { c0 = sub4(bias, 4 * ms); c1 = c0; }
               else { c0 = sub4(acc[0], 8 * ms); c1 = sub4(acc[0], 8 * ms + 4); }
 #define DFN_X3_PARTS(...) \
               _Pragma("unroll") for (int q = 0; q < NPMAX; ++q) \
@@ -466,7 +476,22 @@
 #undef DFN_X3_PARTS
               put4(acc[0], 8 * ms, c0);
               put4(acc[0], 8 * ms + 4, c1);
-              if (from_carry && kc == CIN - 1) asm volatile("s_nop 3");
+              if constexpr (TAILBLK) {
+                if (from_carry) {
+                  __builtin_amdgcn_sched_barrier(0);
+                  asm volatile("s_nop 7");
+                  X3Piece tp[4];
+#pragma unroll
+                  for (int q = 0; q < 4; ++q) tp[q].template A<CIN_RELU>(carry[0], 4 + q);
+#pragma unroll
+                  for (int q = 0; q < 4; ++q) tp[q].B1(pscale2);
+#pragma unroll
+                  for (int q = 0; q < 4; ++q) tp[q].B2(pscale);
+#pragma unroll
+                  for (int q = 0; q < 4; ++q) tp[q].template C<CIN_RELU, P>(Bin[0], CIN / 2, 4 + q, rmax_);
+                }
+              }
+              if (from_carry && kc == CINL - 1) asm volatile("s_nop 3");
               __builtin_amdgcn_sched_barrier(0);
               continue;
             }
@@ -537,7 +562,10 @@
               const f32x16 v = head[nb];
               const bool g1 = (g16 & 1) != 0;
 #pragma unroll
-              for (int c = 0; c < 8; ++c) head[nb][c] = g1 ? v[8 * (c >> 2) + 4 + (c & 3)] : v[8 * (c >> 2) + (c & 3)];
+              for (int c = 0; c < 8; ++c) {
+                if (HALF && c >= 4) head[nb][c] = 0.f;
+                else head[nb][c] = g1 ? v[8 * (c >> 2) + 4 + (c & 3)] : v[8 * (c >> 2) + (c & 3)];
+              }
             }
           }
         }
diff --git a/dfnet_amd/csrc/nerfh_mlp_half.hip b/dfnet_amd/csrc/nerfh_mlp_half.hip
--- /dev/null
+++ b/dfnet_amd/csrc/nerfh_mlp_half.hip
@@ -0,0 +1,3 @@
+#define DFN_MLP_FOLD_TU 1
+#define DFN_MLP_HALF_TU 1
+#include "nerfh_mlp.hip"
```
